# Kaixhin/imitation-learning

Measured on NVIDIA H100. Metric: env_steps_per_s, higher is better.
Workload: dtype f32

## Files before the change

### imitation-learning_b200/csrc/api.cu

```cuda
#include "common.cuh"
#include <cstdlib>

thread_local char g_il_error[512] = "";
int gail_init();
int gmmil_pwil_init();
int gemm_init();
int mlp_init();

extern "C" const char* il_last_error(void) { return g_il_error; }
extern "C" int il_version(void) { return 100; }

extern "C" int il_create(int device, il_handle** out) {
  IL_CHECK(out != nullptr, "il_create: null out");
  int count = 0;
  cudaError_t e = cudaGetDeviceCount(&count);
  if (e != cudaSuccess || count == 0) IL_FAIL("il_create: no CUDA device (%s); this library has no CPU fallback", cudaGetErrorString(e));
  IL_CHECK(device >= 0 && device < count, "il_create: device %d out of range (%d devices)", device, count);
  cudaDeviceProp prop;
  IL_CUDA(cudaGetDeviceProperties(&prop, device));
  IL_CHECK(prop.major == 9 && prop.minor == 0, "il_create: device %d is sm_%d%d; this library is built for sm_90a (H100) only", device, prop.major, prop.minor);
  IL_CUDA(cudaSetDevice(device));
  IL_TRY(gail_init());
  IL_TRY(gmmil_pwil_init());
  IL_TRY(tc_gemm_init());
  IL_TRY(gemm_init());
  IL_TRY(mlp_init());
  il_handle* h = new il_handle();
  h->device = device;
  h->sm_count = prop.multiProcessorCount;
  h->gemm_mode = IL_GEMM_FP32;
  {
    const char* wt = getenv("IL_WIDE_TN");
    h->wide_tn = (wt && wt[0] == '0') ? 0 : 1;
    const char* ff = getenv("IL_FIRST_LAYER_FAST");
    h->first_layer_fast = ff ? atoi(ff) : 2;
    const char* mb = getenv("IL_MASK_BITS");
    h->mask_bits = mb ? atoi(mb) : 2;
    const char* hf = getenv("IL_HEAD_FUSED");
    h->head_fused = (hf && hf[0] == '0') ? 0 : 1;
    const char* ds = getenv("IL_DEBUG_SYNC");
    h->debug_sync = (ds && ds[0] == '1') ? 1 : 0;
    const char* at = getenv("IL_ADAM_TMA");
    h->adam_tma = at ? atoi(at) : 1;
    const char* gt = getenv("IL_GAIL_TILED");
    h->gail_tiled = (gt && gt[0] == '0') ? 0 : 1;
    const char* fl = getenv("IL_TC_FUSE_L1");
    h->tc_fuse_l1 = (fl && fl[0] == '1') ? 1 : 0;
    const char* th = getenv("IL_THIN_HOIST");
    h->thin_hoist = (th && th[0] == '0') ? 0 : 1;
  }
  h->launches = 0;
  h->profiling = 0;
  h->profiled_bytes = 0.0;
  h->eval_graph = nullptr;
  h->build_stream = nullptr;
  *out = h;
  return 0;
}

extern "C" int il_destroy(il_handle* h) {
  if (h) il_eval_release(h);
  if (h && h->build_stream) cudaStreamDestroy(h->build_stream);
  delete h;
  return 0;
}

extern "C" int il_set_gemm_mode(il_handle* h, int mode) {
  IL_CHECK(h, "il_set_gemm_mode: null handle");
  IL_CHECK(mode >= IL_GEMM_FP32 && mode <= IL_GEMM_TF32, "il_set_gemm_mode: bad mode %d", mode);
  h->gemm_mode = mode;
  return 0;
}

extern "C" int64_t il_launch_count(il_handle* h) { return h ? h->launches : -1; }

extern "C" int il_set_option(il_handle* h, const char* name, int value) {
  IL_CHECK(h && name, "il_set_option: null argument");
  if (!strcmp(name, "tc_fuse_l1")) h->tc_fuse_l1 = value;
  else if (!strcmp(name, "gail_tiled")) h->gail_tiled = value;
  else if (!strcmp(name, "adam_tma")) h->adam_tma = value;
  else if (!strcmp(name, "head_fused")) h->head_fused = value;
  else if (!strcmp(name, "mask_bits")) h->mask_bits = value;
  else if (!strcmp(name, "first_layer_fast")) h->first_layer_fast = value;
  else if (!strcmp(name, "wide_tn")) h->wide_tn = value;
  else if (!strcmp(name, "thin_hoist")) h->thin_hoist = value;
  else IL_FAIL("il_set_option: unknown option '%s'", name);
  return 0;
}

extern "C" int il_struct_sizes(int32_t* out) {
  out[0] = (int32_t)sizeof(il_mlp);
  out[1] = (int32_t)sizeof(il_adam);
  out[2] = (int32_t)sizeof(il_batch);
  out[3] = (int32_t)sizeof(il_replay);
  out[4] = (int32_t)sizeof(il_sac_args);
  out[5] = (int32_t)sizeof(il_gail);
  out[6] = (int32_t)sizeof(il_gail_update_args);
  out[7] = (int32_t)sizeof(il_pwil);
  out[8] = (int32_t)sizeof(il_env);
  out[9] = (int32_t)sizeof(il_bc_args);
  out[10] = (int32_t)sizeof(il_eval_args);
  out[11] = (int32_t)sizeof(il_gailx);
  out[12] = (int32_t)sizeof(il_gailx_update_args);
  out[13] = (int32_t)sizeof(il_red);
  out[14] = (int32_t)sizeof(il_red_update_args);
  return 0;
}

extern "C" int il_mlp_param_offsets(const int32_t* dims, int n_layers, int64_t* w_off, int64_t* b_off, int64_t* total) {
  IL_CHECK(dims && n_layers >= 1 && n_layers <= IL_MAX_LAYERS, "il_mlp_param_offsets: bad arguments");
  const MlpOffsets o = mlp_offsets(dims, n_layers);
  for (int l = 0; l < n_layers; ++l) {
    if (w_off) w_off[l] = o.w[l];
    if (b_off) b_off[l] = o.b[l];
  }
  if (total) *total = o.total;
  return 0;
}

extern "C" int il_row_layout(int S, int A, int32_t* off, int32_t* row_len) {
  IL_CHECK(S > 0 && A > 0, "il_row_layout: S=%d A=%d", S, A);
  const RowLayout L = row_layout(S, A);
  if (off) {
    off[0] = L.state; off[1] = L.action; off[2] = L.reward; off[3] = L.next_state;
    off[4] = L.terminal; off[5] = L.timeout; off[6] = L.weight; off[7] = L.step;
  }
  if (row_len) *row_len = L.len;
  return 0;
}

namespace {

__global__ void fill_kernel(float* __restrict__ out, int64_t n, uint64_t seed, uint64_t stream_id, const uint64_t* __restrict__ counter, int normal,
                            const uint64_t* __restrict__ seed_r) {
  const uint64_t base = counter ? *counter : 0ull;
  if (seed_r) { seed = seed_r[blockIdx.y]; out += (int64_t)blockIdx.y * n; }
  const uint2 key = make_uint2((uint32_t)seed, (uint32_t)(seed >> 32));
  for (int64_t q = (int64_t)blockIdx.x * blockDim.x + threadIdx.x; q * 4 < n; q += (int64_t)gridDim.x * blockDim.x) {
    const uint64_t c = base + (uint64_t)q;
    const uint4 r = philox4x32_10(make_uint4((uint32_t)c, (uint32_t)(c >> 32), (uint32_t)stream_id, (uint32_t)(stream_id >> 32)), key);
    float v[4];
    if (normal) {
      const float u0 = 1.f - u32_to_unit(r.x), u1 = u32_to_unit(r.y), u2 = 1.f - u32_to_unit(r.z), u3 = u32_to_unit(r.w);
      const float r0 = sqrtf(-2.f * logf(u0)), r1 = sqrtf(-2.f * logf(u2));
      float s0, c0, s1, c1;
      sincospif(2.f * u1, &s0, &c0);
      sincospif(2.f * u3, &s1, &c1);
      v[0] = r0 * c0; v[1] = r0 * s0; v[2] = r1 * c1; v[3] = r1 * s1;
    } else {
      v[0] = u32_to_unit(r.x); v[1] = u32_to_unit(r.y); v[2] = u32_to_unit(r.z); v[3] = u32_to_unit(r.w);
    }
    for (int j = 0; j < 4; ++j)
      if (q * 4 + j < n) out[q * 4 + j] = v[j];
  }
}

constexpr int BETA_ATTEMPTS = 16;

__device__ float log_gamma_mt(float a, uint64_t c, uint64_t stream_id, uint32_t tag, uint2 key, float* boost_u) {
  const float d = a - 1.f / 3.f, cc = 1.f / sqrtf(9.f * d);
  for (int k = 0; k < BETA_ATTEMPTS; ++k) {
    const uint4 q = philox4x32_10(make_uint4((uint32_t)c, (uint32_t)(c >> 32), (uint32_t)stream_id, (uint32_t)(stream_id >> 32) ^ (tag | (uint32_t)k)), key);
    if (k == 0) *boost_u = 1.f - u32_to_unit(q.w);
    const float x = sqrtf(-2.f * logf(1.f - u32_to_unit(q.x))) * cospif(2.f * u32_to_unit(q.y));
    const float t = fmaf(cc, x, 1.f);
    if (t <= 0.f) continue;
    const float lt = logf(t), v = t * t * t;
    if (logf(1.f - u32_to_unit(q.z)) < 0.5f * x * x + d - d * v + 3.f * d * lt) return logf(d) + 3.f * lt;
  }
  return logf(d);
}

__global__ void beta_fill_kernel(float* __restrict__ out, int64_t total, int64_t n, const float* __restrict__ alpha_r, uint64_t seed, uint64_t stream_id,
                                 const uint64_t* __restrict__ counter, const uint64_t* __restrict__ seed_r) {
  const uint64_t base = counter ? *counter : 0ull;
  if (seed_r) { seed = seed_r[blockIdx.y]; out += (int64_t)blockIdx.y * n; total = n; }
  const uint2 key = make_uint2((uint32_t)seed, (uint32_t)(seed >> 32));
  for (int64_t i = (int64_t)blockIdx.x * blockDim.x + threadIdx.x; i < total; i += (int64_t)gridDim.x * blockDim.x) {
    const uint64_t c = base + (uint64_t)(i >> 2);
    const uint32_t lane = (uint32_t)(i & 3);
    const float alpha = alpha_r[seed_r ? (int64_t)blockIdx.y : i / n];
    float v;
    if (alpha == 1.f) {
      const uint4 q = philox4x32_10(make_uint4((uint32_t)c, (uint32_t)(c >> 32), (uint32_t)stream_id, (uint32_t)(stream_id >> 32)), key);
      v = u32_to_unit(lane == 0 ? q.x : lane == 1 ? q.y : lane == 2 ? q.z : q.w);
    } else if (!(alpha > 0.f)) {
      v = __int_as_float(0x7fc00000);
    } else {
      const float a = alpha < 1.f ? alpha + 1.f : alpha;
      float ux, uy;
      float lx = log_gamma_mt(a, c, stream_id, 0x80000000u | (lane << 5), key, &ux);
      float ly = log_gamma_mt(a, c, stream_id, 0x80000000u | (lane << 5) | 16u, key, &uy);
      if (alpha < 1.f) { lx += logf(ux) / alpha; ly += logf(uy) / alpha; }
      const float t = ly - lx;
      v = t >= 0.f ? 1.f / (1.f + expf(t)) : 1.f - 1.f / (1.f + expf(-t));
    }
    out[i] = v;
  }
}

__global__ void counter_add_kernel(uint64_t* c, uint64_t inc) { *c += inc; }

dim3 rng_grid(il_handle* h, int64_t units, int R) {
  int64_t blocks = (units + 255) / 256;
  const int64_t cap = (int64_t)h->sm_count * 16 / R;
  if (blocks > cap) blocks = cap;
  if (blocks < 1) blocks = 1;
  return dim3((unsigned)blocks, (unsigned)R);
}

int fill(il_handle* h, float* out, int64_t n, uint64_t seed, uint64_t stream_id, const uint64_t* counter, void* stream, int normal) {
  IL_CHECK(h && out && n >= 0, "il_fill: bad argument");
  if (n == 0) return 0;
  int64_t blocks = (n / 4 + 255) / 256;
  if (blocks > (int64_t)h->sm_count * 16) blocks = (int64_t)h->sm_count * 16;
  if (blocks < 1) blocks = 1;
  IL_LAUNCH(h, fill_kernel, (unsigned)blocks, 256, 0, (cudaStream_t)stream, out, n, seed, stream_id, counter, normal, nullptr);
  return 0;
}

int fill_r(il_handle* h, float* out, int R, int64_t n_per_replica, const uint64_t* seed_r, uint64_t stream_id, const uint64_t* counter, void* stream, int normal) {
  IL_CHECK(h && out && seed_r && R > 0 && R <= IL_MAX_GRID_Y && n_per_replica >= 0, "il_fill_%s_r: bad argument (R = %d)", normal ? "normal" : "uniform", R);
  if (n_per_replica == 0) return 0;
  IL_LAUNCH(h, fill_kernel, rng_grid(h, (n_per_replica + 3) / 4, R), 256, 0, (cudaStream_t)stream, out, n_per_replica, 0ull, stream_id, counter, normal, seed_r);
  return 0;
}

}

extern "C" int il_fill_normal(il_handle* h, float* out, int64_t n, uint64_t seed, uint64_t stream_id, const uint64_t* counter, void* stream) {
  return fill(h, out, n, seed, stream_id, counter, stream, 1);
}
extern "C" int il_fill_uniform(il_handle* h, float* out, int64_t n, uint64_t seed, uint64_t stream_id, const uint64_t* counter, void* stream) {
  return fill(h, out, n, seed, stream_id, counter, stream, 0);
}
extern "C" int il_fill_normal_r(il_handle* h, float* out, int R, int64_t n_per_replica, const uint64_t* seed_r, uint64_t stream_id, const uint64_t* counter, void* stream) {
  return fill_r(h, out, R, n_per_replica, seed_r, stream_id, counter, stream, 1);
}
extern "C" int il_fill_uniform_r(il_handle* h, float* out, int R, int64_t n_per_replica, const uint64_t* seed_r, uint64_t stream_id, const uint64_t* counter, void* stream) {
  return fill_r(h, out, R, n_per_replica, seed_r, stream_id, counter, stream, 0);
}
extern "C" int il_fill_beta(il_handle* h, float* out, int R, int64_t n_per_replica, const float* alpha_r, uint64_t seed, uint64_t stream_id, const uint64_t* counter,
                            void* stream) {
  IL_CHECK(h && out && alpha_r && R > 0 && n_per_replica >= 0, "il_fill_beta: bad argument");
  const int64_t total = (int64_t)R * n_per_replica;
  if (total == 0) return 0;
  int64_t blocks = (total + 255) / 256;
  if (blocks > (int64_t)h->sm_count * 16) blocks = (int64_t)h->sm_count * 16;
  IL_LAUNCH(h, beta_fill_kernel, (unsigned)blocks, 256, 0, (cudaStream_t)stream, out, total, n_per_replica, alpha_r, seed, stream_id, counter, nullptr);
  return 0;
}
extern "C" int il_fill_beta_r(il_handle* h, float* out, int R, int64_t n_per_replica, const float* alpha_r, const uint64_t* seed_r, uint64_t stream_id,
                              const uint64_t* counter, void* stream) {
  IL_CHECK(h && out && alpha_r && seed_r && R > 0 && R <= IL_MAX_GRID_Y && n_per_replica >= 0, "il_fill_beta_r: bad argument (R = %d)", R);
  if (n_per_replica == 0) return 0;
  IL_LAUNCH(h, beta_fill_kernel, rng_grid(h, n_per_replica, R), 256, 0, (cudaStream_t)stream, out, n_per_replica, n_per_replica, alpha_r, 0ull, stream_id, counter, seed_r);
  return 0;
}
extern "C" int il_counter_add(il_handle* h, uint64_t* counter, uint64_t inc, void* stream) {
  IL_CHECK(h && counter, "il_counter_add: null argument");
  IL_LAUNCH(h, counter_add_kernel, 1, 1, 0, (cudaStream_t)stream, counter, inc);
  return 0;
}
```

### imitation-learning_b200/csrc/common.cuh

```cuda
#pragma once
#include <cuda_runtime.h>
#include <stdint.h>
#include <stdio.h>
#include <string.h>

#include <vector>

#include "../../include/il_b200.h"

#define IL_MAX_GRID_Y 65535

struct ProfiledLaunch {
  cudaEvent_t start, stop;
  double flops;
  double bytes;
};
struct il_handle {
  int device;
  int sm_count;
  int gemm_mode;
  int thin_hoist;
  int wide_tn;
  int first_layer_fast;
  int mask_bits;
  int head_fused;
  int debug_sync;
  int adam_tma;
  int gail_tiled;
  int tc_fuse_l1;
  long long launches;
  int profiling;
  std::vector<ProfiledLaunch> profiled;
  double profiled_bytes;
  void* eval_graph;
  cudaStream_t build_stream;
};
void il_eval_release(il_handle* h);

extern thread_local char g_il_error[512];

#define IL_FAIL(...)                                     \
  do {                                                   \
    snprintf(g_il_error, sizeof(g_il_error), __VA_ARGS__); \
    return 1;                                            \
  } while (0)

#define IL_CHECK(cond, ...)        \
  do {                             \
    if (!(cond)) IL_FAIL(__VA_ARGS__); \
  } while (0)

#define IL_CUDA(expr)                                                                             \
  do {                                                                                            \
    cudaError_t _e = (expr);                                                                      \
    if (_e != cudaSuccess) IL_FAIL("%s failed: %s (%s:%d)", #expr, cudaGetErrorString(_e), __FILE__, __LINE__); \
  } while (0)

#define IL_LAUNCH(h, kernel, grid, block, smem, stream, ...)                                      \
  do {                                                                                            \
    kernel<<<(grid), (block), (smem), (cudaStream_t)(stream)>>>(__VA_ARGS__);                     \
    (h)->launches++;                                                                              \
    cudaError_t _e = cudaPeekAtLastError();                                                       \
    if (_e != cudaSuccess) IL_FAIL("launch of %s failed: %s (%s:%d)", #kernel, cudaGetErrorString(_e), __FILE__, __LINE__); \
  } while (0)

#define IL_TRY(expr)          \
  do {                        \
    int _r = (expr);          \
    if (_r != 0) return _r;   \
  } while (0)

__host__ __device__ static inline int64_t il_align_up(int64_t x, int64_t a) { return (x + a - 1) / a * a; }

struct RowLayout {
  int state, action, reward, next_state, terminal, timeout, weight, step, len;
};
__host__ __device__ inline RowLayout row_layout(int S, int A) {
  RowLayout L;
  L.state = 0;
  L.action = S;
  L.reward = S + A;
  L.next_state = S + A + 1;
  L.terminal = 2 * S + A + 1;
  L.timeout = L.terminal + 1;
  L.weight = L.terminal + 2;
  L.step = L.terminal + 3;
  L.len = (2 * S + A + 5 + 3) / 4 * 4;
  return L;
}

struct MlpOffsets {
  int64_t w[IL_MAX_LAYERS], b[IL_MAX_LAYERS], total;
};
__host__ __device__ static inline MlpOffsets mlp_offsets(const int32_t* dims, int n_layers) {
  MlpOffsets o;
  int64_t off = 0;
  for (int l = 0; l < n_layers; ++l) {
    o.w[l] = off;
    off = il_align_up(off + (int64_t)dims[l + 1] * dims[l], 4);
    o.b[l] = off;
    off = il_align_up(off + dims[l + 1], 4);
  }
  o.total = il_align_up(off, 32);
  return o;
}

__device__ __forceinline__ float act_apply(float x, int act) {
  if (act == IL_ACT_RELU) return fmaxf(x, 0.f);
  if (act == IL_ACT_TANH) return tanhf(x);
  return 1.f / (1.f + expf(-x));
}
__device__ __forceinline__ float act_grad_from_output(float y, int act) {
  if (act == IL_ACT_RELU) return y > 0.f ? 1.f : 0.f;
  if (act == IL_ACT_TANH) return 1.f - y * y;
  return y * (1.f - y);
}
__device__ __forceinline__ float softplusf(float x) {
  return x > 20.f ? x : log1pf(expf(x));
}
__device__ __forceinline__ float sigmoidf(float x) { return 1.f / (1.f + expf(-x)); }

__device__ __forceinline__ float warp_sum(float v) {
#pragma unroll
  for (int o = 16; o > 0; o >>= 1) v += __shfl_xor_sync(0xffffffffu, v, o);
  return v;
}
__device__ __forceinline__ float warp_max(float v) {
#pragma unroll
  for (int o = 16; o > 0; o >>= 1) v = fmaxf(v, __shfl_xor_sync(0xffffffffu, v, o));
  return v;
}
__device__ __forceinline__ float block_sum(float v, float* red) {
  const int lane = threadIdx.x & 31, warp = threadIdx.x >> 5, nw = (blockDim.x + 31) >> 5;
  v = warp_sum(v);
  __syncthreads();
  if (lane == 0) red[warp] = v;
  __syncthreads();
  float r = 0.f;
  if (warp == 0) {
    r = lane < nw ? red[lane] : 0.f;
    r = warp_sum(r);
    if (lane == 0) red[0] = r;
  }
  __syncthreads();
  return red[0];
}

__device__ __forceinline__ uint4 philox4x32_10(uint4 ctr, uint2 key) {
  const uint32_t M0 = 0xD2511F53u, M1 = 0xCD9E8D57u, W0 = 0x9E3779B9u, W1 = 0xBB67AE85u;
#pragma unroll
  for (int i = 0; i < 10; ++i) {
    const uint32_t hi0 = __umulhi(M0, ctr.x), lo0 = M0 * ctr.x;
    const uint32_t hi1 = __umulhi(M1, ctr.z), lo1 = M1 * ctr.z;
    ctr = make_uint4(hi1 ^ ctr.y ^ key.x, lo1, hi0 ^ ctr.w ^ key.y, lo0);
    key.x += W0;
    key.y += W1;
  }
  return ctr;
}
__device__ __forceinline__ float u32_to_unit(uint32_t x) { return (float)(x >> 8) * (1.0f / 16777216.0f); }

struct GemmArgs {
  const float* A;
  int64_t a_gs;
  int a_gdiv, lda, a_kmajor;
  const float* B;
  int64_t b_gs;
  int b_gdiv, ldb, b_kmajor;
  float* C;
  int64_t c_gs;
  int ldc;
  const float* bias;
  int64_t bias_gs;
  int act;
  const float* mask;
  int64_t mask_gs;
  int ldmask, mask_act;
  float* colsum;
  int64_t colsum_gs;
  int accumulate;
  int M, N, K, G;
  const uint32_t* mask_bits;
  int64_t mask_bits_gs;
  uint32_t* bits_out;
  int64_t bits_out_gs;
};
int launch_gemm(il_handle* h, const GemmArgs& a, cudaStream_t stream);
bool gemm_uses_tc(const il_handle* h, const GemmArgs& a);
bool gemm_first_layer_emits_bits(const il_handle* h, const GemmArgs& a);
double gemm_algorithmic_bytes(const GemmArgs& a, bool stores_c);
int profile_open(il_handle* h, ProfiledLaunch* pl, double flops, double bytes, cudaStream_t stream);
int profile_close(il_handle* h, ProfiledLaunch* pl, cudaStream_t stream);

bool tc_gemm_eligible(const GemmArgs& a);
int launch_tc_gemm(il_handle* h, const GemmArgs& a, cudaStream_t stream);
int tc_gemm_init();
struct TcFuseL1 {
  const float* x;
  int64_t x_gs;
  int x_gdiv, x_ld, x_k;
  const float* w1;
  const float* b1;
  int64_t gs;
  float* store;
  int64_t store_gs;
};
bool tc_head_fusable(const il_handle* h, const GemmArgs& a, int head_n);
bool tc_l1_fusable(const il_handle* h, const GemmArgs& a, int x_k);
bool tc_dx_head_fusable(const il_handle* h, const GemmArgs& a, int head_n);
int launch_tc_gemm_dx_head(il_handle* h, const GemmArgs& a, const float* w, int64_t w_gs, int w_ns, int head_n, float* out, int64_t out_gs, cudaStream_t stream);
int launch_tc_gemm_head(il_handle* h, const GemmArgs& a, const float* head_w, const float* head_b, int64_t head_gs, int head_n, float* head_out, int64_t head_out_gs, int store_c,
                        cudaStream_t stream, const TcFuseL1* l1 = nullptr);
```

### imitation-learning_b200/csrc/mlp.cu

```cuda
#include "mlp.cuh"

#include <math.h>

constexpr int HB_MAXN = 8;
struct HeadBwdArgs {
  const float* dout; int64_t dout_gs; int dout_gdiv, ld_dout;
  const float* w; int64_t w_gs;
  const float* y; int64_t y_gs;
  float* dz; int64_t dz_gs;
  float* dw; float* db; float* db_prev; int64_t g_gs;
  int n, H, Nh;
};
int launch_head_backward(il_handle* h, const HeadBwdArgs& a, int G, cudaStream_t stream);
int launch_head_dx_bits(il_handle* h, const HeadBwdArgs& a, const uint32_t* bits, int64_t bits_gs, int G, cudaStream_t stream);

int mlp_validate(const il_mlp* m, const char* what) {
  IL_CHECK(m != nullptr && m->params != nullptr, "%s: null mlp", what);
  IL_CHECK(m->n_layers >= 1 && m->n_layers <= IL_MAX_LAYERS, "%s: n_layers %d out of range", what, m->n_layers);
  IL_CHECK(m->activation >= 0 && m->activation <= 2, "%s: bad activation %d", what, m->activation);
  for (int l = 0; l <= m->n_layers; ++l) IL_CHECK(m->dims[l] > 0, "%s: dims[%d] = %d", what, l, m->dims[l]);
  const MlpOffsets o = mlp_offsets(m->dims, m->n_layers);
  IL_CHECK(m->stride >= o.total - 31 && m->stride % 4 == 0, "%s: stride %lld too small / unaligned for %lld parameters", what, (long long)m->stride, (long long)o.total);
  IL_CHECK((reinterpret_cast<uintptr_t>(m->params) & 15) == 0, "%s: params not 16-byte aligned", what);
  return 0;
}

int mlp_max_hidden(const il_mlp* m) {
  int mx = 1;
  for (int l = 1; l <= m->n_layers; ++l) mx = m->dims[l] > mx ? m->dims[l] : mx;
  return mx;
}

static int64_t mlp_bits_bytes(const il_mlp* m, int G, int n, int l) {
  return m->dims[l + 1] % 32 == 0 ? il_align_up((int64_t)G * n * (m->dims[l + 1] / 32) * 4, 256) : 0;
}

int64_t mlp_acts_bytes(const il_mlp* m, int G, int n) {
  int64_t b = 0;
  for (int l = 0; l + 1 < m->n_layers; ++l) b += il_align_up((int64_t)G * n * m->dims[l + 1] * 4, 256) + mlp_bits_bytes(m, G, n, l);
  return b;
}

char* mlp_acts_carve(const il_mlp* m, int G, int n, char* ws, MlpActs* acts) {
  for (int l = 0; l < IL_MAX_LAYERS; ++l) { acts->hid[l] = nullptr; acts->bits[l] = nullptr; acts->bits_valid[l] = false; }
  for (int l = 0; l + 1 < m->n_layers; ++l) {
    acts->hid[l] = reinterpret_cast<float*>(ws);
    ws += il_align_up((int64_t)G * n * m->dims[l + 1] * 4, 256);
    if (mlp_bits_bytes(m, G, n, l)) {
      acts->bits[l] = reinterpret_cast<uint32_t*>(ws);
      ws += mlp_bits_bytes(m, G, n, l);
    }
  }
  return ws;
}

int mlp_forward(il_handle* h, const il_mlp* m, int G, int n, MatView X, MlpActs& acts, float* out, int64_t out_gs, int ld_out, cudaStream_t stream, int keep) {
  const MlpOffsets o = mlp_offsets(m->dims, m->n_layers);
  const int L = m->n_layers;
  const bool keep_hidden = keep != MLP_KEEP_NONE;
  const bool want_bits = h->mask_bits && keep_hidden && m->activation == IL_ACT_RELU;
  for (int l = 0; l < IL_MAX_LAYERS; ++l) acts.bits_valid[l] = false;
  auto layer_args = [&](int l) {
    GemmArgs a{};
    if (l == 0) { a.A = X.ptr; a.a_gs = X.gs; a.a_gdiv = X.gdiv; a.lda = X.ld; }
    else { a.A = acts.hid[l - 1]; a.a_gs = (int64_t)n * m->dims[l]; a.a_gdiv = 1; a.lda = m->dims[l]; }
    a.a_kmajor = 1;
    a.B = m->params + o.w[l]; a.b_gs = m->stride; a.b_gdiv = 1; a.ldb = m->dims[l]; a.b_kmajor = 1;
    a.bias = m->params + o.b[l]; a.bias_gs = m->stride;
    if (l == L - 1) { a.C = out; a.c_gs = out_gs; a.ldc = ld_out; a.act = -1; }
    else { a.C = acts.hid[l]; a.c_gs = (int64_t)n * m->dims[l + 1]; a.ldc = m->dims[l + 1]; a.act = m->activation; }
    a.M = n; a.N = m->dims[l + 1]; a.K = m->dims[l]; a.G = G;
    return a;
  };
  const bool head_shape = L >= 2 && m->activation == IL_ACT_RELU && ld_out == m->dims[L] && out_gs == (int64_t)n * m->dims[L];
  for (int l = 0; l < L; ++l) {
    if (head_shape && l == L - 2) {
      GemmArgs a = layer_args(l);
      if (tc_head_fusable(h, a, m->dims[L])) {
        const bool bits = want_bits && keep == MLP_KEEP_MASKS && acts.bits[l] && m->dims[L] <= HB_MAXN;
        if (bits) { a.bits_out = acts.bits[l]; a.bits_out_gs = (int64_t)n * (m->dims[l + 1] / 32); acts.bits_valid[l] = true; }
        IL_TRY(launch_tc_gemm_head(h, a, m->params + o.w[L - 1], m->params + o.b[L - 1], m->stride, m->dims[L], out, out_gs, keep_hidden && !bits ? 1 : 0, stream));
        return 0;
      }
    }
    if (head_shape && l == 0 && L == 3) {
      GemmArgs a1 = layer_args(1);
      a1.A = nullptr; a1.a_gs = 0; a1.a_gdiv = 1; a1.lda = m->dims[1];
      if (tc_head_fusable(h, a1, m->dims[L]) && tc_l1_fusable(h, a1, m->dims[0])) {
        TcFuseL1 f{};
        f.x = X.ptr; f.x_gs = X.gs; f.x_gdiv = X.gdiv; f.x_ld = X.ld; f.x_k = m->dims[0];
        f.w1 = m->params + o.w[0]; f.b1 = m->params + o.b[0]; f.gs = m->stride;
        f.store = keep_hidden ? acts.hid[0] : nullptr; f.store_gs = (int64_t)n * m->dims[1];
        IL_TRY(launch_tc_gemm_head(h, a1, m->params + o.w[L - 1], m->params + o.b[L - 1], m->stride, m->dims[L], out, out_gs, keep_hidden ? 1 : 0, stream, &f));
        return 0;
      }
    }
    GemmArgs a = layer_args(l);
    if (want_bits && l + 1 < L && acts.bits[l] && gemm_first_layer_emits_bits(h, a)) {
      a.bits_out = acts.bits[l]; a.bits_out_gs = (int64_t)n * (m->dims[l + 1] / 32);
      acts.bits_valid[l] = true;
    }
    IL_TRY(launch_gemm(h, a, stream));
  }
  return 0;
}

static bool head_backward_eligible(const il_mlp* m, int n, int64_t grad_stride) {
  const int L = m->n_layers, H = m->dims[L - 1], Nh = m->dims[L];
  return m->activation == IL_ACT_RELU && Nh <= HB_MAXN && H % 4 == 0 && n <= 1024 && grad_stride % 4 == 0 && m->stride % 4 == 0;
}

int mlp_backward(il_handle* h, const il_mlp* m, int G, int n, MatView X, const MlpActs& acts, MatView dOut, float* grads, int64_t grad_stride,
                 float* dX, int64_t dx_gs, int ld_dx, int dx_col0, int dx_cols, float* tmpA, float* tmpB, cudaStream_t stream) {
  const MlpOffsets o = mlp_offsets(m->dims, m->n_layers);
  const int L = m->n_layers;
  MatView dZ = dOut;
  float* next_tmp = tmpA;
  bool bias_done = false;
  for (int l = L - 1; l >= 0; --l) {
    MatView Xin = l == 0 ? X : MatView{acts.hid[l - 1], (int64_t)n * m->dims[l], 1, m->dims[l]};
    if (l == L - 1 && l > 0 && grads && h->head_fused && head_backward_eligible(m, n, grad_stride)) {
      HeadBwdArgs a{};
      a.dout = dZ.ptr; a.dout_gs = dZ.gs; a.dout_gdiv = dZ.gdiv; a.ld_dout = dZ.ld;
      a.w = m->params + o.w[l]; a.w_gs = m->stride;
      a.y = acts.hid[l - 1]; a.y_gs = (int64_t)n * m->dims[l];
      a.dz = next_tmp; a.dz_gs = (int64_t)n * m->dims[l];
      a.dw = grads + o.w[l]; a.db = grads + o.b[l]; a.db_prev = grads + o.b[l - 1]; a.g_gs = grad_stride;
      a.n = n; a.H = m->dims[l]; a.Nh = m->dims[l + 1];
      IL_TRY(launch_head_backward(h, a, G, stream));
      dZ = MatView{next_tmp, (int64_t)n * m->dims[l], 1, m->dims[l]};
      next_tmp = next_tmp == tmpA ? tmpB : tmpA;
      bias_done = true;
      continue;
    }
    if (l == L - 1 && l > 0 && !grads && acts.bits_valid[l - 1] && m->dims[l + 1] <= HB_MAXN) {
      HeadBwdArgs a{};
      a.dout = dZ.ptr; a.dout_gs = dZ.gs; a.dout_gdiv = dZ.gdiv; a.ld_dout = dZ.ld;
      a.w = m->params + o.w[l]; a.w_gs = m->stride;
      a.dz = next_tmp; a.dz_gs = (int64_t)n * m->dims[l];
      a.n = n; a.H = m->dims[l]; a.Nh = m->dims[l + 1];
      IL_TRY(launch_head_dx_bits(h, a, acts.bits[l - 1], (int64_t)n * (m->dims[l] / 32), G, stream));
      dZ = MatView{next_tmp, (int64_t)n * m->dims[l], 1, m->dims[l]};
      next_tmp = next_tmp == tmpA ? tmpB : tmpA;
      continue;
    }
    if (grads) {
      GemmArgs a{};
      a.A = dZ.ptr; a.a_gs = dZ.gs; a.a_gdiv = dZ.gdiv; a.lda = dZ.ld; a.a_kmajor = 0;
      a.B = Xin.ptr; a.b_gs = Xin.gs; a.b_gdiv = Xin.gdiv; a.ldb = Xin.ld; a.b_kmajor = 0;
      a.C = grads + o.w[l]; a.c_gs = grad_stride; a.ldc = m->dims[l]; a.act = -1;
      if (!bias_done) { a.colsum = grads + o.b[l]; a.colsum_gs = grad_stride; }
      bias_done = false;
      a.M = m->dims[l + 1]; a.N = m->dims[l]; a.K = n; a.G = G;
      IL_TRY(launch_gemm(h, a, stream));
    }
    if (l > 0) {
      GemmArgs a{};
      a.A = dZ.ptr; a.a_gs = dZ.gs; a.a_gdiv = dZ.gdiv; a.lda = dZ.ld; a.a_kmajor = 1;
      a.B = m->params + o.w[l]; a.b_gs = m->stride; a.b_gdiv = 1; a.ldb = m->dims[l]; a.b_kmajor = 0;
      a.C = next_tmp; a.c_gs = (int64_t)n * m->dims[l]; a.ldc = m->dims[l]; a.act = -1;
      a.mask_act = m->activation;
      a.M = n; a.N = m->dims[l]; a.K = m->dims[l + 1]; a.G = G;
      if (acts.bits_valid[l - 1] && m->activation == IL_ACT_RELU && gemm_uses_tc(h, a)) {
        a.mask_bits = acts.bits[l - 1]; a.mask_bits_gs = (int64_t)n * (m->dims[l] / 32);
        if (h->mask_bits >= 2 && l == 1 && !grads && dX && ld_dx == dx_cols && dx_gs == (int64_t)n * dx_cols && tc_dx_head_fusable(h, a, dx_cols)) {
          a.C = nullptr;
          IL_TRY(launch_tc_gemm_dx_head(h, a, m->params + o.w[0] + dx_col0, m->stride, m->dims[0], dx_cols, dX, dx_gs, stream));
          return 0;
        }
      } else {
        a.mask = acts.hid[l - 1]; a.mask_gs = (int64_t)n * m->dims[l]; a.ldmask = m->dims[l];
      }
      IL_TRY(launch_gemm(h, a, stream));
      dZ = MatView{next_tmp, (int64_t)n * m->dims[l], 1, m->dims[l]};
      next_tmp = next_tmp == tmpA ? tmpB : tmpA;
    } else if (dX) {
      GemmArgs a{};
      a.A = dZ.ptr; a.a_gs = dZ.gs; a.a_gdiv = dZ.gdiv; a.lda = dZ.ld; a.a_kmajor = 1;
      a.B = m->params + o.w[0] + dx_col0; a.b_gs = m->stride; a.b_gdiv = 1; a.ldb = m->dims[0]; a.b_kmajor = 0;
      a.C = dX; a.c_gs = dx_gs; a.ldc = ld_dx; a.act = -1;
      a.M = n; a.N = dx_cols; a.K = m->dims[1]; a.G = G;
      IL_TRY(launch_gemm(h, a, stream));
    }
  }
  return 0;
}

namespace {

__global__ void actor_head_kernel(const HeadFwdArgs p) {
  const int64_t row = (int64_t)blockIdx.x * blockDim.x + threadIdx.x;
  if (row >= (int64_t)p.R * p.n) return;
  const int r = (int)(row / p.n), i = (int)(row % p.n);
  const int A = p.A;
  const float* hd = p.head + row * 2 * A;
  float* act_row = p.action ? p.action + (int64_t)r * p.action_rs + (int64_t)i * p.ld_action : nullptr;
  if (p.copy_src && act_row) {
    const float* src = p.copy_src + (int64_t)r * p.copy_rs + (int64_t)i * p.copy_ld;
    for (int j = 0; j < p.copy_cols; ++j) act_row[j - p.copy_cols] = __ldg(src + j);
  }
  const float keep = p.zero_mask ? 1.f - __ldg(p.zero_mask + (int64_t)r * p.zero_mask_rs + (int64_t)i * p.zero_mask_ld) : 1.f;
  const float LOG_SQRT_2PI = 0.91893853320467274178f, LOG2 = 0.69314718055994530942f;
  const float A_LO = (float)(-1.0 + 1e-6), A_HI = (float)(1.0 - 1e-6);
  float sum_ladj = 0.f, sum_nlp = 0.f;
  const bool want_lp = p.log_prob != nullptr && (p.eps != nullptr || p.given != nullptr);
  for (int j = 0; j < A; ++j) {
    const float mu = hd[j];
    const float ls = fminf(fmaxf(hd[A + j], -20.f), 2.f);
    if (p.mean) p.mean[row * A + j] = mu;
    if (p.log_std) p.log_std[row * A + j] = ls;
    float x, a;
    const float sd = expf(ls);
    if (p.given) {
      a = fminf(fmaxf(p.given[row * A + j], A_LO), A_HI);
      x = atanhf(a);
    } else if (p.eps) {
      x = __fadd_rn(mu, __fmul_rn(sd, p.eps[row * A + j]));
      a = tanhf(x);
    } else {
      x = mu;
      a = tanhf(mu);
    }
    if (act_row && !p.given) act_row[j] = keep * a;
    if (want_lp) {
      const float var = __fmul_rn(sd, sd);
      const float diff = __fsub_rn(x, mu);
      float nlp = __fdiv_rn(-__fmul_rn(diff, diff), __fmul_rn(2.f, var));
      nlp = __fsub_rn(__fsub_rn(nlp, logf(sd)), LOG_SQRT_2PI);
      const float ladj = __fmul_rn(2.f, __fsub_rn(__fsub_rn(LOG2, x), softplusf(__fmul_rn(-2.f, x))));
      sum_nlp += nlp;
      sum_ladj += ladj;
    }
  }
  if (want_lp) p.log_prob[row] = __fadd_rn(__fsub_rn(0.f, sum_ladj), sum_nlp);
}

struct SmallFwdArgs {
  il_mlp m;
  MlpOffsets o;
  const float* X;
  int64_t x_gs;
  int x_gdiv, ldx, n, maxd;
  float* out;
  int tanh_first;
};
template <int NR>
__global__ void __launch_bounds__(256) mlp_small_forward_kernel(const SmallFwdArgs p) {
  extern __shared__ __align__(16) float sm[];
  const int g = blockIdx.x, r0 = blockIdx.y * NR, tid = threadIdx.x, warp = tid >> 5, lane = tid & 31;
  const int nr = min(NR, p.n - r0), L = p.m.n_layers, maxd = p.maxd;
  float* bufs[2] = {sm, sm + NR * maxd};
  const float* X = p.X + (int64_t)(g / p.x_gdiv) * p.x_gs;
  for (int idx = tid; idx < NR * p.m.dims[0]; idx += 256) {
    const int r = idx / p.m.dims[0], k = idx % p.m.dims[0];
    bufs[0][r * maxd + k] = r < nr ? __ldg(X + (int64_t)(r0 + r) * p.ldx + k) : 0.f;
  }
  const float* prm = p.m.params + (int64_t)g * p.m.stride;
  __syncthreads();
  for (int l = 0; l < L; ++l) {
    const int in = p.m.dims[l], od = p.m.dims[l + 1];
    const float* W = prm + p.o.w[l];
    const float* bias = prm + p.o.b[l];
    const float* xin = bufs[l & 1];
    float* xout = bufs[(l + 1) & 1];
    const bool vec = (in % 4 == 0) && (p.m.stride % 4 == 0);
    if (NR == 1 && vec && in <= 16) {
      for (int o = tid; o < od; o += 256) {
        const float4* wr = reinterpret_cast<const float4*>(W + (int64_t)o * in);
        float4 w4[4];
#pragma unroll
        for (int q = 0; q < 4; ++q) w4[q] = 4 * q < in ? __ldg(wr + q) : make_float4(0.f, 0.f, 0.f, 0.f);
        float v = __ldg(bias + o);
#pragma unroll
        for (int q = 0; q < 4; ++q)
          if (4 * q < in) {
            const float4 x4 = *reinterpret_cast<const float4*>(xin + 4 * q);
            v = fmaf(w4[q].x, x4.x, fmaf(w4[q].y, x4.y, fmaf(w4[q].z, x4.z, fmaf(w4[q].w, x4.w, v))));
          }
        if (l < L - 1) v = act_apply(v, p.m.activation);
        xout[o] = v;
      }
      __syncthreads();
      continue;
    }
    if (NR == 1 && vec && in % 128 == 0 && in <= 256) {
      const int kv = in >> 7;
      float4 x4[2];
#pragma unroll
      for (int v = 0; v < 2; ++v) x4[v] = v < kv ? *reinterpret_cast<const float4*>(xin + v * 128 + lane * 4) : make_float4(0.f, 0.f, 0.f, 0.f);
      for (int o0 = warp * 8; o0 < od; o0 += 64) {
        float4 w4[8][2];
#pragma unroll
        for (int u = 0; u < 8; ++u)
#pragma unroll
          for (int v = 0; v < 2; ++v)
            w4[u][v] = (o0 + u < od && v < kv) ? __ldg(reinterpret_cast<const float4*>(W + (int64_t)(o0 + u) * in + v * 128 + lane * 4)) : make_float4(0.f, 0.f, 0.f, 0.f);
        float a8[8];
#pragma unroll
        for (int u = 0; u < 8; ++u) {
          float t = 0.f;
#pragma unroll
          for (int v = 0; v < 2; ++v) t = fmaf(w4[u][v].x, x4[v].x, fmaf(w4[u][v].y, x4[v].y, fmaf(w4[u][v].z, x4[v].z, fmaf(w4[u][v].w, x4[v].w, t))));
          a8[u] = warp_sum(t);
        }
        if (lane < 8 && o0 + lane < od) {
          float v = a8[0];
#pragma unroll
          for (int u = 1; u < 8; ++u) v = lane == u ? a8[u] : v;
          v += __ldg(bias + o0 + lane);
          if (l < L - 1) v = act_apply(v, p.m.activation);
          xout[o0 + lane] = v;
        }
      }
      __syncthreads();
      continue;
    }
    if (NR == 1 && vec) {
      for (int o0 = warp * 4; o0 < od; o0 += 32) {
        float a4[4] = {0.f, 0.f, 0.f, 0.f};
        for (int k = lane * 4; k < in; k += 128) {
          const float4 x4 = *reinterpret_cast<const float4*>(xin + k);
          float4 w4[4];
#pragma unroll
          for (int u = 0; u < 4; ++u) w4[u] = o0 + u < od ? __ldg(reinterpret_cast<const float4*>(W + (int64_t)(o0 + u) * in + k)) : make_float4(0.f, 0.f, 0.f, 0.f);
#pragma unroll
          for (int u = 0; u < 4; ++u) a4[u] = fmaf(w4[u].x, x4.x, fmaf(w4[u].y, x4.y, fmaf(w4[u].z, x4.z, fmaf(w4[u].w, x4.w, a4[u]))));
        }
#pragma unroll
        for (int u = 0; u < 4; ++u) a4[u] = warp_sum(a4[u]);
        if (lane < 4 && o0 + lane < od) {
          float v = (lane == 0 ? a4[0] : lane == 1 ? a4[1] : lane == 2 ? a4[2] : a4[3]) + __ldg(bias + o0 + lane);
          if (l < L - 1) v = act_apply(v, p.m.activation);
          xout[o0 + lane] = v;
        }
      }
      __syncthreads();
      continue;
    }
    for (int o = warp; o < od; o += 8) {
      float acc[NR];
#pragma unroll
      for (int r = 0; r < NR; ++r) acc[r] = 0.f;
      const float* wr = W + (int64_t)o * in;
      if (vec) {
        for (int k = lane * 4; k < in; k += 128) {
          const float4 w4 = __ldg(reinterpret_cast<const float4*>(wr + k));
#pragma unroll
          for (int r = 0; r < NR; ++r) {
            const float4 x4 = *reinterpret_cast<const float4*>(xin + r * maxd + k);
            acc[r] = fmaf(w4.x, x4.x, fmaf(w4.y, x4.y, fmaf(w4.z, x4.z, fmaf(w4.w, x4.w, acc[r]))));
          }
        }
      } else {
        for (int k = lane; k < in; k += 32) {
          const float w = __ldg(wr + k);
#pragma unroll
          for (int r = 0; r < NR; ++r) acc[r] = fmaf(w, xin[r * maxd + k], acc[r]);
        }
      }
#pragma unroll
      for (int r = 0; r < NR; ++r) acc[r] = warp_sum(acc[r]);
      if (lane == 0) {
        const float b = __ldg(bias + o);
#pragma unroll
        for (int r = 0; r < NR; ++r) {
          float v = acc[r] + b;
          if (l < L - 1) v = act_apply(v, p.m.activation);
          xout[r * maxd + o] = v;
        }
      }
    }
    __syncthreads();
  }
  const int od = p.m.dims[L];
  const float* fin = bufs[L & 1];
  if (p.tanh_first > 0) {
    const int A = p.tanh_first;
    for (int idx = tid; idx < nr * A; idx += 256) {
      const int r = idx / A, o = idx % A;
      p.out[((int64_t)g * p.n + r0 + r) * A + o] = tanhf(fin[r * maxd + o]);
    }
    return;
  }
  for (int idx = tid; idx < nr * od; idx += 256) {
    const int r = idx / od, o = idx % od;
    p.out[((int64_t)g * p.n + r0 + r) * od + o] = fin[r * maxd + o];
  }
}

struct AdamReplicas {
  const double* lr_r;
  const double* wd_r;
  const float* tau_r;
  int64_t rf;
  float inv_rf;
  int R;
};
struct AdamCoef { float step_size, decay, tau, one_minus_tau; };
constexpr int ADAM_MAX_REPLICAS = 2048;
__device__ __forceinline__ void adam_fill_table(AdamCoef* tab, const AdamReplicas& rp, double lr, double wd, double beta1_d, const int64_t* step, float tau) {
  if (!rp.R) return;
  const double bc1 = 1.0 - pow(beta1_d, (double)*step);
  for (int r = threadIdx.x; r < rp.R; r += blockDim.x) {
    const double l = rp.lr_r ? rp.lr_r[r] : lr, w = rp.wd_r ? rp.wd_r[r] : wd;
    const float t = rp.tau_r ? rp.tau_r[r] : tau;
    tab[r] = AdamCoef{(float)(l / bc1), w != 0.0 ? (float)(1.0 - l * w) : 1.f, t, (float)(1.0 - (double)t)};
  }
}
__device__ __forceinline__ int adam_replica(int64_t f, const AdamReplicas& rp) {
  int r = (int)((float)f * rp.inv_rf);
  if ((int64_t)r * rp.rf > f) --r;
  else if ((int64_t)(r + 1) * rp.rf <= f) ++r;
  return r;
}

__global__ void adam_kernel(float* __restrict__ p, const float* __restrict__ g, float* __restrict__ m, float* __restrict__ v, const int64_t* __restrict__ step,
                            double lr, double beta1_d, double beta2_d, double eps_d, double wd, int64_t n, float* __restrict__ target, float tau, float one_minus_tau,
                            const AdamReplicas rp) {
  extern __shared__ AdamCoef adam_tab[];
  __shared__ float s_step_size, s_bc2_sqrt;
  if (threadIdx.x == 0) {
    const double t = (double)*step;
    const double bc1 = 1.0 - pow(beta1_d, t), bc2 = 1.0 - pow(beta2_d, t);
    s_step_size = (float)(lr / bc1);
    s_bc2_sqrt = (float)sqrt(bc2);
  }
  adam_fill_table(adam_tab, rp, lr, wd, beta1_d, step, tau);
  __syncthreads();
  const float step_size = s_step_size, bc2_sqrt = s_bc2_sqrt;
  const float decay = (float)(1.0 - lr * wd), w1 = (float)(1.0 - beta1_d), w2 = (float)(1.0 - beta2_d);
  const float beta2 = (float)beta2_d, eps = (float)eps_d;
  const bool has_wd = wd != 0.0;
  auto upd = [&](float& pi, float& mi, float& vi, float gi, float ss, float dc, bool wdf) {
    if (wdf) pi = __fmul_rn(pi, dc);
    mi = __fadd_rn(mi, __fmul_rn(w1, __fsub_rn(gi, mi)));
    vi = __fadd_rn(__fmul_rn(vi, beta2), __fmul_rn(__fmul_rn(w2, gi), gi));
    const float denom = __fadd_rn(__fdiv_rn(sqrtf(vi), bc2_sqrt), eps);
    pi = __fadd_rn(pi, __fmul_rn(-ss, __fdiv_rn(mi, denom)));
  };
  const int64_t n4 = n >> 2;
  for (int64_t i = (int64_t)blockIdx.x * blockDim.x + threadIdx.x; i < n4; i += (int64_t)gridDim.x * blockDim.x) {
    float ss = step_size, dc = decay, ta = tau, omt = one_minus_tau;
    bool wdf = has_wd;
    if (rp.R) {
      const AdamCoef c = adam_tab[adam_replica(i << 2, rp)];
      ss = c.step_size; dc = c.decay; wdf = c.decay != 1.f; ta = c.tau; omt = c.one_minus_tau;
    }
    float4 pv = reinterpret_cast<float4*>(p)[i], mv = reinterpret_cast<float4*>(m)[i], vv = reinterpret_cast<float4*>(v)[i];
    const float4 gv = reinterpret_cast<const float4*>(g)[i];
    upd(pv.x, mv.x, vv.x, gv.x, ss, dc, wdf); upd(pv.y, mv.y, vv.y, gv.y, ss, dc, wdf); upd(pv.z, mv.z, vv.z, gv.z, ss, dc, wdf); upd(pv.w, mv.w, vv.w, gv.w, ss, dc, wdf);
    reinterpret_cast<float4*>(p)[i] = pv; reinterpret_cast<float4*>(m)[i] = mv; reinterpret_cast<float4*>(v)[i] = vv;
    if (target) {
      const float tau = ta, one_minus_tau = omt;
      float4 tv = reinterpret_cast<float4*>(target)[i];
      tv.x = __fadd_rn(__fmul_rn(tv.x, tau), __fmul_rn(one_minus_tau, pv.x)); tv.y = __fadd_rn(__fmul_rn(tv.y, tau), __fmul_rn(one_minus_tau, pv.y));
      tv.z = __fadd_rn(__fmul_rn(tv.z, tau), __fmul_rn(one_minus_tau, pv.z)); tv.w = __fadd_rn(__fmul_rn(tv.w, tau), __fmul_rn(one_minus_tau, pv.w));
      reinterpret_cast<float4*>(target)[i] = tv;
    }
  }
  for (int64_t i = (n4 << 2) + (int64_t)blockIdx.x * blockDim.x + threadIdx.x; i < n; i += (int64_t)gridDim.x * blockDim.x) {
    float pi = p[i], mi = m[i], vi = v[i];
    upd(pi, mi, vi, g[i], step_size, decay, has_wd);
    p[i] = pi; m[i] = mi; v[i] = vi;
    if (target) target[i] = __fadd_rn(__fmul_rn(target[i], tau), __fmul_rn(one_minus_tau, pi));
  }
}

constexpr int ADAM_STREAMS = 5;
constexpr int ADAM_CONSUMERS = 256;
template <int TILE, int STAGES> constexpr int adam_tma_smem() { return STAGES * ADAM_STREAMS * TILE * 4 + 2 * STAGES * 8 + 64; }
__device__ __forceinline__ void adam_mbar_wait(uint32_t bar, uint32_t parity) {
  asm volatile(
      "{\n\t.reg .pred q;\n\t"
      "ADAM_WAIT:\n\t"
      "mbarrier.try_wait.parity.shared::cta.b64 q, [%0], %1;\n\t"
      "@q bra ADAM_DONE;\n\t"
      "bra ADAM_WAIT;\n\t"
      "ADAM_DONE:\n\t}" ::"r"(bar), "r"(parity) : "memory");
}
template <int TILE, int STAGES>
__global__ void __launch_bounds__(ADAM_CONSUMERS + 32) adam_tma_kernel(float* __restrict__ p, const float* __restrict__ g, float* __restrict__ m, float* __restrict__ v,
                                                                      const int64_t* __restrict__ step, double lr, double beta1_d, double beta2_d, double eps_d, double wd, int64_t n,
                                                                      float* __restrict__ target, float tau, float one_minus_tau, const AdamReplicas rp) {
  extern __shared__ __align__(128) uint8_t adam_smem[];
  float* buf = reinterpret_cast<float*>(adam_smem);
  AdamCoef* tab = reinterpret_cast<AdamCoef*>(adam_smem + adam_tma_smem<TILE, STAGES>());
  const uint32_t smem0 = (uint32_t)__cvta_generic_to_shared(buf);
  const uint32_t full0 = smem0 + (uint32_t)(STAGES * ADAM_STREAMS * TILE * 4), done0 = full0 + 8u * STAGES;
  __shared__ float s_step_size, s_bc2_sqrt;
  const int tid = threadIdx.x;
  adam_fill_table(tab, rp, lr, wd, beta1_d, step, tau);
  if (tid == 0) {
    const double t = (double)*step;
    s_step_size = (float)(lr / (1.0 - pow(beta1_d, t)));
    s_bc2_sqrt = (float)sqrt(1.0 - pow(beta2_d, t));
    for (int s_ = 0; s_ < STAGES; ++s_) {
      asm volatile("mbarrier.init.shared::cta.b64 [%0], 1;" ::"r"(full0 + 8u * s_));
      asm volatile("mbarrier.init.shared::cta.b64 [%0], %1;" ::"r"(done0 + 8u * s_), "r"(ADAM_CONSUMERS));
    }
    asm volatile("fence.mbarrier_init.release.cluster;" ::: "memory");
  }
  __syncthreads();
  const int64_t n_tiles = (n + TILE - 1) / TILE;
  const int n_streams = target ? 5 : 4;
  auto tile_floats = [&](int64_t tile) { const int64_t left = n - tile * TILE; return (int)(left < TILE ? left : TILE); };
  const int64_t my_tiles = blockIdx.x < n_tiles ? (n_tiles - blockIdx.x + gridDim.x - 1) / gridDim.x : 0;
  if (tid >= ADAM_CONSUMERS) {
    if (tid != ADAM_CONSUMERS) return;
    auto issue_loads = [&](int64_t k) {
      const int64_t tile = blockIdx.x + k * gridDim.x;
      const int stage = (int)(k % STAGES);
      const uint32_t bytes = (uint32_t)tile_floats(tile) * 4u, bar = full0 + 8u * stage;
      asm volatile("mbarrier.arrive.expect_tx.shared::cta.b64 _, [%0], %1;" ::"r"(bar), "r"(bytes * (uint32_t)n_streams) : "memory");
      const float* src[5] = {p, g, m, v, target};
      for (int q = 0; q < n_streams; ++q)
        asm volatile("cp.async.bulk.shared::cluster.global.mbarrier::complete_tx::bytes [%0], [%1], %2, [%3];" ::"r"(smem0 + (uint32_t)((stage * ADAM_STREAMS + q) * TILE * 4)),
                     "l"(src[q] + tile * TILE), "r"(bytes), "r"(bar) : "memory");
    };
    for (int64_t k = 0; k < STAGES - 1 && k < my_tiles; ++k) issue_loads(k);
    for (int64_t k = 0; k < my_tiles; ++k) {
      const int stage = (int)(k % STAGES);
      const int64_t tile = blockIdx.x + k * gridDim.x;
      if (k + STAGES - 1 < my_tiles) {
        if (k > 0) asm volatile("cp.async.bulk.wait_group.read 0;" ::: "memory");
        issue_loads(k + STAGES - 1);
      }
      adam_mbar_wait(done0 + 8u * stage, (uint32_t)((k / STAGES) & 1));
      const uint32_t bytes = (uint32_t)tile_floats(tile) * 4u;
      float* dst[5] = {p, nullptr, m, v, target};
      for (int q = 0; q < n_streams; ++q) {
        if (!dst[q]) continue;
        asm volatile("cp.async.bulk.global.shared::cta.bulk_group [%0], [%1], %2;" ::"l"(dst[q] + tile * TILE), "r"(smem0 + (uint32_t)((stage * ADAM_STREAMS + q) * TILE * 4)), "r"(bytes)
                     : "memory");
      }
      asm volatile("cp.async.bulk.commit_group;" ::: "memory");
    }
    asm volatile("cp.async.bulk.wait_group 0;" ::: "memory");
    return;
  }
  const float step_size = s_step_size, bc2_sqrt = s_bc2_sqrt;
  const float decay = (float)(1.0 - lr * wd), w1 = (float)(1.0 - beta1_d), w2 = (float)(1.0 - beta2_d), beta2 = (float)beta2_d, eps = (float)eps_d;
  const bool has_wd = wd != 0.0;
  auto upd = [&](float& pi, float& mi, float& vi, float gi, float ss, float dc, bool wdf) {
    if (wdf) pi = __fmul_rn(pi, dc);
    mi = __fadd_rn(mi, __fmul_rn(w1, __fsub_rn(gi, mi)));
    vi = __fadd_rn(__fmul_rn(vi, beta2), __fmul_rn(__fmul_rn(w2, gi), gi));
    const float denom = __fadd_rn(__fdiv_rn(sqrtf(vi), bc2_sqrt), eps);
    pi = __fadd_rn(pi, __fmul_rn(-ss, __fdiv_rn(mi, denom)));
  };
  for (int64_t k = 0; k < my_tiles; ++k) {
    const int stage = (int)(k % STAGES);
    const int64_t tile = blockIdx.x + k * gridDim.x;
    adam_mbar_wait(full0 + 8u * stage, (uint32_t)((k / STAGES) & 1));
    const int nf4 = tile_floats(tile) >> 2;
    float4* sp = reinterpret_cast<float4*>(buf + (stage * ADAM_STREAMS + 0) * TILE);
    const float4* sg = reinterpret_cast<const float4*>(buf + (stage * ADAM_STREAMS + 1) * TILE);
    float4* smm = reinterpret_cast<float4*>(buf + (stage * ADAM_STREAMS + 2) * TILE);
    float4* sv = reinterpret_cast<float4*>(buf + (stage * ADAM_STREAMS + 3) * TILE);
    float4* stg = reinterpret_cast<float4*>(buf + (stage * ADAM_STREAMS + 4) * TILE);
    for (int i = tid; i < nf4; i += ADAM_CONSUMERS) {
      float ss = step_size, dc = decay, ta = tau, omt = one_minus_tau;
      bool wdf = has_wd;
      if (rp.R) {
        const AdamCoef c = tab[adam_replica(tile * TILE + 4 * i, rp)];
        ss = c.step_size; dc = c.decay; wdf = c.decay != 1.f; ta = c.tau; omt = c.one_minus_tau;
      }
      float4 pv = sp[i], mv = smm[i], vv = sv[i];
      const float4 gv = sg[i];
      upd(pv.x, mv.x, vv.x, gv.x, ss, dc, wdf); upd(pv.y, mv.y, vv.y, gv.y, ss, dc, wdf); upd(pv.z, mv.z, vv.z, gv.z, ss, dc, wdf); upd(pv.w, mv.w, vv.w, gv.w, ss, dc, wdf);
      sp[i] = pv; smm[i] = mv; sv[i] = vv;
      if (target) {
        const float tau = ta, one_minus_tau = omt;
        float4 tv = stg[i];
        tv.x = __fadd_rn(__fmul_rn(tv.x, tau), __fmul_rn(one_minus_tau, pv.x)); tv.y = __fadd_rn(__fmul_rn(tv.y, tau), __fmul_rn(one_minus_tau, pv.y));
        tv.z = __fadd_rn(__fmul_rn(tv.z, tau), __fmul_rn(one_minus_tau, pv.z)); tv.w = __fadd_rn(__fmul_rn(tv.w, tau), __fmul_rn(one_minus_tau, pv.w));
        stg[i] = tv;
      }
    }
    asm volatile("fence.proxy.async.shared::cta;" ::: "memory");
    asm volatile("mbarrier.arrive.shared::cta.b64 _, [%0];" ::"r"(done0 + 8u * stage) : "memory");
  }
}

template <int TILE, int STAGES>
static int launch_adam_tma(il_handle* h, int ctas_per_sm, float* params, const float* grads, const il_adam* opt, int64_t n, cudaStream_t stream, float* polyak_target, float polyak_factor,
                           const AdamReplicas& rp) {
  static bool attr_set = false;
  if (!attr_set) {
    IL_CUDA(cudaFuncSetAttribute(adam_tma_kernel<TILE, STAGES>, cudaFuncAttributeMaxDynamicSharedMemorySize, adam_tma_smem<TILE, STAGES>() + ADAM_MAX_REPLICAS * (int)sizeof(AdamCoef)));
    attr_set = true;
  }
  const size_t smem = (size_t)adam_tma_smem<TILE, STAGES>() + (size_t)rp.R * sizeof(AdamCoef);
  IL_LAUNCH(h, (adam_tma_kernel<TILE, STAGES>), h->sm_count * ctas_per_sm, ADAM_CONSUMERS + 32, smem, stream, params, grads, opt->m, opt->v, opt->step, opt->lr, opt->beta1,
            opt->beta2, opt->eps, opt->weight_decay, n, polyak_target, polyak_factor, (float)(1.0 - (double)polyak_factor), rp);
  return 0;
}
constexpr int ADAM_TMA_MIN_TILES = 4096;


template <int NH>
__global__ void __launch_bounds__(256, 2) head_backward_kernel(const HeadBwdArgs p) {
  extern __shared__ __align__(16) float hb_sm[];
  const int g = blockIdx.y, n0 = blockIdx.x * 256, tid = threadIdx.x, tc = tid & 63, tr = tid >> 6, col = n0 + tc * 4;
  float* dos = hb_sm;
  float* red = hb_sm + p.n * HB_MAXN;
  const float* dout = p.dout + (int64_t)(g / p.dout_gdiv) * p.dout_gs;
  const bool active = col < p.H;
  const float* Y = p.y + (int64_t)g * p.y_gs + col;
  float4 yv[4], yn[4];
  auto fetch = [&](float4 (&dst)[4], int b0) {
#pragma unroll
    for (int u = 0; u < 4; ++u) {
      const int b = b0 + 4 * u;
      dst[u] = (active && b < p.n) ? __ldg(reinterpret_cast<const float4*>(Y + (int64_t)b * p.H)) : make_float4(0.f, 0.f, 0.f, 0.f);
    }
  };
  fetch(yv, tr);
  for (int i = tid; i < p.n * HB_MAXN; i += 256) {
    const int b = i / HB_MAXN, j = i % HB_MAXN;
    dos[i] = j < p.Nh ? __ldg(dout + (int64_t)b * p.ld_dout + j) : 0.f;
  }
  float4 w[NH];
#pragma unroll
  for (int j = 0; j < NH; ++j) w[j] = (active && j < p.Nh) ? __ldg(reinterpret_cast<const float4*>(p.w + (int64_t)g * p.w_gs + (int64_t)j * p.H + col)) : make_float4(0.f, 0.f, 0.f, 0.f);
  __syncthreads();
  float4 dw[NH], cs = make_float4(0.f, 0.f, 0.f, 0.f);
#pragma unroll
  for (int j = 0; j < NH; ++j) dw[j] = make_float4(0.f, 0.f, 0.f, 0.f);
  if (active) {
    float* DZ = p.dz + (int64_t)g * p.dz_gs + col;
    for (int b0 = tr; b0 < p.n; b0 += 16) {
      fetch(yn, b0 + 16);
#pragma unroll
      for (int u = 0; u < 4; ++u) {
        const int b = b0 + 4 * u;
        if (b >= p.n) continue;
        float dj[NH];
        if (NH == 1) dj[0] = dos[b * HB_MAXN];
        else {
          const float4 d0 = *reinterpret_cast<const float4*>(dos + b * HB_MAXN), d1 = *reinterpret_cast<const float4*>(dos + b * HB_MAXN + 4);
          const float t[8] = {d0.x, d0.y, d0.z, d0.w, d1.x, d1.y, d1.z, d1.w};
#pragma unroll
          for (int j = 0; j < NH; ++j) dj[j] = t[j];
        }
        float4 z = make_float4(0.f, 0.f, 0.f, 0.f);
#pragma unroll
        for (int j = 0; j < NH; ++j) {
          z.x = fmaf(dj[j], w[j].x, z.x); z.y = fmaf(dj[j], w[j].y, z.y); z.z = fmaf(dj[j], w[j].z, z.z); z.w = fmaf(dj[j], w[j].w, z.w);
          dw[j].x = fmaf(dj[j], yv[u].x, dw[j].x); dw[j].y = fmaf(dj[j], yv[u].y, dw[j].y); dw[j].z = fmaf(dj[j], yv[u].z, dw[j].z); dw[j].w = fmaf(dj[j], yv[u].w, dw[j].w);
        }
        z.x = yv[u].x > 0.f ? z.x : 0.f; z.y = yv[u].y > 0.f ? z.y : 0.f; z.z = yv[u].z > 0.f ? z.z : 0.f; z.w = yv[u].w > 0.f ? z.w : 0.f;
        cs.x += z.x; cs.y += z.y; cs.z += z.z; cs.w += z.w;
        *reinterpret_cast<float4*>(DZ + (int64_t)b * p.H) = z;
      }
#pragma unroll
      for (int u = 0; u < 4; ++u) yv[u] = yn[u];
    }
  }
  float4* r4 = reinterpret_cast<float4*>(red);
#pragma unroll
  for (int j = 0; j < NH; ++j) r4[(tr * (HB_MAXN + 1) + j) * 64 + tc] = dw[j];
  r4[(tr * (HB_MAXN + 1) + HB_MAXN) * 64 + tc] = cs;
  __syncthreads();
  if (tr == 0 && active) {
#pragma unroll
    for (int j = 0; j <= HB_MAXN; ++j) {
      if ((j < NH && j < p.Nh) || j == HB_MAXN) {
        float4 a = r4[(0 * (HB_MAXN + 1) + j) * 64 + tc];
#pragma unroll
        for (int q = 1; q < 4; ++q) {
          const float4 t = r4[(q * (HB_MAXN + 1) + j) * 64 + tc];
          a.x += t.x; a.y += t.y; a.z += t.z; a.w += t.w;
        }
        float* dst = j == HB_MAXN ? p.db_prev + (int64_t)g * p.g_gs + col : p.dw + (int64_t)g * p.g_gs + (int64_t)j * p.H + col;
        *reinterpret_cast<float4*>(dst) = a;
      }
    }
  }
  if (blockIdx.x == 0 && tid < p.Nh) {
    float sacc = 0.f;
    for (int b = 0; b < p.n; ++b) sacc += dos[b * HB_MAXN + tid];
    p.db[(int64_t)g * p.g_gs + tid] = sacc;
  }
}

__global__ void tick_kernel(int64_t* s0, int64_t* s1, int64_t* s2) {
  if (s0) *s0 += 1;
  if (s1) *s1 += 1;
  if (s2) *s2 += 1;
}

__global__ void polyak_kernel(float* __restrict__ t, const float* __restrict__ o, int64_t n, float tau, float one_minus_tau) {
  for (int64_t i = (int64_t)blockIdx.x * blockDim.x + threadIdx.x; i < n; i += (int64_t)gridDim.x * blockDim.x)
    t[i] = __fadd_rn(__fmul_rn(t[i], tau), __fmul_rn(one_minus_tau, o[i]));
}

__global__ void split_twin_kernel(const float* __restrict__ q, float* __restrict__ q1, float* __restrict__ q2, int R, int n) {
  const int64_t i = (int64_t)blockIdx.x * blockDim.x + threadIdx.x;
  if (i >= (int64_t)R * n) return;
  const int r = (int)(i / n), b = (int)(i % n);
  if (q1) q1[i] = q[((int64_t)2 * r) * n + b];
  if (q2) q2[i] = q[((int64_t)2 * r + 1) * n + b];
}

__global__ void concat_kernel(const float* __restrict__ s, int64_t s_rs, int ld_s, int S, const float* __restrict__ a, int64_t a_rs, int ld_a, int A,
                              float* __restrict__ x, int R, int n) {
  const int64_t idx = (int64_t)blockIdx.x * blockDim.x + threadIdx.x;
  const int d = S + A;
  if (idx >= (int64_t)R * n * d) return;
  const int j = (int)(idx % d);
  const int64_t row = idx / d;
  const int r = (int)(row / n), i = (int)(row % n);
  x[idx] = j < S ? s[(int64_t)r * s_rs + (int64_t)i * ld_s + j] : a[(int64_t)r * a_rs + (int64_t)i * ld_a + (j - S)];
}

inline int ew_blocks(int64_t n, int threads, int sm_count) {
  int64_t b = (n + threads - 1) / threads;
  const int64_t cap = (int64_t)sm_count * 16;
  return (int)(b < 1 ? 1 : (b > cap ? cap : b));
}

}

int launch_actor_head(il_handle* h, const HeadFwdArgs& a, cudaStream_t stream) {
  const int64_t rows = (int64_t)a.R * a.n;
  IL_LAUNCH(h, actor_head_kernel, (unsigned)((rows + 127) / 128), 128, 0, stream, a);
  return 0;
}

int launch_adam(il_handle* h, float* params, const float* grads, const il_adam* opt, int64_t n, cudaStream_t stream, float* polyak_target, float polyak_factor,
                const float* polyak_r) {
  IL_CHECK(opt->m && opt->v && opt->step, "adam: null state");
  IL_CHECK(((reinterpret_cast<uintptr_t>(params) | reinterpret_cast<uintptr_t>(grads) | reinterpret_cast<uintptr_t>(opt->m) | reinterpret_cast<uintptr_t>(opt->v) |
             reinterpret_cast<uintptr_t>(polyak_target)) & 15) == 0, "adam: buffers must be 16-byte aligned");
  AdamReplicas rp{opt->lr_r, opt->weight_decay_r, polyak_target ? polyak_r : nullptr, 0, 0.f, 0};
  if (rp.lr_r || rp.wd_r || rp.tau_r) {
    const int64_t rf = opt->replica_floats;
    IL_CHECK(rf > 0 && rf % 4 == 0 && n % rf == 0, "adam: per-replica hyper-parameters need replica_floats (%lld) > 0, a multiple of 4 dividing n = %lld", (long long)rf, (long long)n);
    IL_CHECK(n / rf <= ADAM_MAX_REPLICAS, "adam: %lld replicas with per-replica hyper-parameters exceed the limit of %d per buffer", (long long)(n / rf), ADAM_MAX_REPLICAS);
    rp.rf = rf; rp.inv_rf = 1.f / (float)rf; rp.R = (int)(n / rf);
  }
  if (h->adam_tma && n % 4 == 0 && n >= (int64_t)ADAM_TMA_MIN_TILES * h->sm_count * 2) {
    const int variant = h->adam_tma;
    switch (variant) {
      case 2: return launch_adam_tma<4096, 2>(h, 1, params, grads, opt, n, stream, polyak_target, polyak_factor, rp);
      case 3: return launch_adam_tma<2048, 3>(h, 1, params, grads, opt, n, stream, polyak_target, polyak_factor, rp);
      case 4: return launch_adam_tma<1024, 4>(h, 2, params, grads, opt, n, stream, polyak_target, polyak_factor, rp);
      case 5: return launch_adam_tma<1024, 3>(h, 3, params, grads, opt, n, stream, polyak_target, polyak_factor, rp);
      case 6: return launch_adam_tma<512, 4>(h, 4, params, grads, opt, n, stream, polyak_target, polyak_factor, rp);
      case 7: return launch_adam_tma<2048, 4>(h, 1, params, grads, opt, n, stream, polyak_target, polyak_factor, rp);
      default: return launch_adam_tma<2048, 2>(h, 2, params, grads, opt, n, stream, polyak_target, polyak_factor, rp);
    }
  }
  IL_LAUNCH(h, adam_kernel, ew_blocks(n / 4 + 1, 256, h->sm_count), 256, (size_t)rp.R * sizeof(AdamCoef), stream, params, grads, opt->m, opt->v, opt->step, opt->lr, opt->beta1, opt->beta2,
            opt->eps, opt->weight_decay, n, polyak_target, polyak_factor, (float)(1.0 - (double)polyak_factor), rp);
  return 0;
}

namespace {
template <int NH, int U>
__global__ void __launch_bounds__(256) head_dx_bits_kernel(const HeadBwdArgs p, const uint32_t* __restrict__ bits, int64_t bits_gs) {
  const int g = blockIdx.y, tid = threadIdx.x, tc = tid & 63, tr = tid >> 6, col = blockIdx.x * 256 + tc * 4;
  if (col >= p.H) return;
  const float* __restrict__ dout = p.dout + (int64_t)(g / p.dout_gdiv) * p.dout_gs;
  const uint32_t* __restrict__ bw = bits + (int64_t)g * bits_gs + (col >> 5);
  const int sh = col & 31, wpr = p.H >> 5;
  float4 w[NH];
#pragma unroll
  for (int j = 0; j < NH; ++j) w[j] = j < p.Nh ? __ldg(reinterpret_cast<const float4*>(p.w + (int64_t)g * p.w_gs + (int64_t)j * p.H + col)) : make_float4(0.f, 0.f, 0.f, 0.f);
  float* __restrict__ dz = p.dz + (int64_t)g * p.dz_gs + col;
  for (int b0 = tr; b0 < p.n; b0 += 4 * U) {
    uint32_t m[U];
    float d[U][NH];
#pragma unroll
    for (int u = 0; u < U; ++u) {
      const int b = b0 + 4 * u;
      m[u] = b < p.n ? __ldg(bw + (int64_t)b * wpr) >> sh : 0u;
#pragma unroll
      for (int j = 0; j < NH; ++j) d[u][j] = (j < p.Nh && b < p.n) ? __ldg(dout + (int64_t)b * p.ld_dout + j) : 0.f;
    }
#pragma unroll
    for (int u = 0; u < U; ++u) {
      const int b = b0 + 4 * u;
      if (b >= p.n) break;
      float4 v = make_float4(0.f, 0.f, 0.f, 0.f);
#pragma unroll
      for (int j = 0; j < NH; ++j)
        if (j < p.Nh) { v.x = fmaf(d[u][j], w[j].x, v.x); v.y = fmaf(d[u][j], w[j].y, v.y); v.z = fmaf(d[u][j], w[j].z, v.z); v.w = fmaf(d[u][j], w[j].w, v.w); }
      v.x = m[u] & 1u ? v.x : 0.f; v.y = m[u] & 2u ? v.y : 0.f; v.z = m[u] & 4u ? v.z : 0.f; v.w = m[u] & 8u ? v.w : 0.f;
      *reinterpret_cast<float4*>(dz + (int64_t)b * p.H) = v;
    }
  }
}
}

int launch_head_dx_bits(il_handle* h, const HeadBwdArgs& a, const uint32_t* bits, int64_t bits_gs, int G, cudaStream_t stream) {
  IL_CHECK(a.H % 32 == 0 && a.Nh <= HB_MAXN && (reinterpret_cast<uintptr_t>(a.w) & 15) == 0 && a.w_gs % 4 == 0 && (reinterpret_cast<uintptr_t>(a.dz) & 15) == 0 && a.dz_gs % 4 == 0,
           "head_dx_bits: H=%d Nh=%d or unaligned buffers", a.H, a.Nh);
  if (a.Nh == 1) IL_LAUNCH(h, (head_dx_bits_kernel<1, 8>), dim3((a.H + 255) / 256, G), 256, 0, stream, a, bits, bits_gs);
  else IL_LAUNCH(h, (head_dx_bits_kernel<HB_MAXN, 4>), dim3((a.H + 255) / 256, G), 256, 0, stream, a, bits, bits_gs);
  return 0;
}

int launch_head_backward(il_handle* h, const HeadBwdArgs& a, int G, cudaStream_t stream) {
  const size_t smem = ((size_t)a.n * HB_MAXN + 4 * (HB_MAXN + 1) * 64 * 4) * sizeof(float);
  if (a.Nh == 1) IL_LAUNCH(h, head_backward_kernel<1>, dim3((a.H + 255) / 256, G), 256, smem, stream, a);
  else IL_LAUNCH(h, head_backward_kernel<HB_MAXN>, dim3((a.H + 255) / 256, G), 256, smem, stream, a);
  return 0;
}

int mlp_init() {
  IL_CUDA(cudaFuncSetAttribute(head_backward_kernel<1>, cudaFuncAttributeMaxDynamicSharedMemorySize, (1024 * HB_MAXN + 4 * (HB_MAXN + 1) * 64 * 4) * 4));
  IL_CUDA(cudaFuncSetAttribute(head_backward_kernel<HB_MAXN>, cudaFuncAttributeMaxDynamicSharedMemorySize, (1024 * HB_MAXN + 4 * (HB_MAXN + 1) * 64 * 4) * 4));
  return 0;
}

int launch_tick(il_handle* h, int64_t* s0, int64_t* s1, int64_t* s2, cudaStream_t stream) {
  IL_LAUNCH(h, tick_kernel, 1, 1, 0, stream, s0, s1, s2);
  return 0;
}

int mlp_small_forward(il_handle* h, const il_mlp* m, int G, int n, MatView X, float* out, cudaStream_t stream, int tanh_first) {
  SmallFwdArgs a;
  a.m = *m; a.o = mlp_offsets(m->dims, m->n_layers);
  a.X = X.ptr; a.x_gs = X.gs; a.x_gdiv = X.gdiv; a.ldx = X.ld; a.n = n; a.out = out; a.tanh_first = tanh_first;
  int maxd = 4;
  for (int l = 0; l <= m->n_layers; ++l) maxd = m->dims[l] > maxd ? m->dims[l] : maxd;
  a.maxd = (maxd + 3) / 4 * 4;
  if (n == 1) {
    IL_LAUNCH(h, mlp_small_forward_kernel<1>, dim3(G, 1), 256, (size_t)2 * 1 * a.maxd * 4, stream, a);
  } else {
    IL_CHECK((size_t)2 * 8 * a.maxd * 4 <= 48 * 1024, "mlp_small_forward: layer width %d too large", maxd);
    IL_LAUNCH(h, mlp_small_forward_kernel<8>, dim3(G, (n + 7) / 8), 256, (size_t)2 * 8 * a.maxd * 4, stream, a);
  }
  return 0;
}

extern "C" int il_adam_step(il_handle* h, float* params, const float* grads, const il_adam* opt, int64_t n, void* stream) {
  IL_CHECK(h && params && grads && opt, "il_adam_step: null argument");
  IL_TRY(launch_tick(h, opt->step, nullptr, nullptr, (cudaStream_t)stream));
  return launch_adam(h, params, grads, opt, n, (cudaStream_t)stream);
}

extern "C" int il_adam_step_polyak(il_handle* h, float* params, const float* grads, const il_adam* opt, int64_t n, float* target, float polyak_factor, void* stream) {
  IL_CHECK(h && params && grads && opt && target, "il_adam_step_polyak: null argument");
  IL_TRY(launch_tick(h, opt->step, nullptr, nullptr, (cudaStream_t)stream));
  return launch_adam(h, params, grads, opt, n, (cudaStream_t)stream, target, polyak_factor);
}

extern "C" int il_adam_step_polyak_r(il_handle* h, float* params, const float* grads, const il_adam* opt, int64_t n, float* target, const float* polyak_r, void* stream) {
  IL_CHECK(h && params && grads && opt && target && polyak_r, "il_adam_step_polyak_r: null argument");
  IL_TRY(launch_tick(h, opt->step, nullptr, nullptr, (cudaStream_t)stream));
  return launch_adam(h, params, grads, opt, n, (cudaStream_t)stream, target, 0.f, polyak_r);
}

extern "C" int il_polyak(il_handle* h, float* target, const float* online, int64_t n, float polyak_factor, void* stream) {
  IL_CHECK(h && target && online && n >= 0, "il_polyak: bad argument");
  if (n == 0) return 0;
  IL_LAUNCH(h, polyak_kernel, ew_blocks(n, 256, h->sm_count), 256, 0, (cudaStream_t)stream, target, online, n, polyak_factor, (float)(1.0 - (double)polyak_factor));
  return 0;
}

extern "C" int64_t il_actor_workspace_bytes(const il_mlp* actor, int R, int n) {
  return mlp_acts_bytes(actor, R, n) + il_align_up((int64_t)R * n * actor->dims[actor->n_layers] * 4, 256);
}

extern "C" int il_actor_forward(il_handle* h, const il_mlp* actor, int R, int n, const float* states, int64_t states_rs, int ld_states, const float* eps,
                                const float* given_action, float* action, float* log_prob, float* mean, float* log_std, void* workspace, int64_t workspace_bytes,
                                void* stream) {
  IL_CHECK(h && states && workspace, "il_actor_forward: null argument");
  IL_TRY(mlp_validate(actor, "il_actor_forward"));
  IL_CHECK(R > 0 && n > 0, "il_actor_forward: R=%d n=%d", R, n);
  const int out = actor->dims[actor->n_layers];
  IL_CHECK(out % 2 == 0, "il_actor_forward: head size %d is not 2*A", out);
  IL_CHECK(workspace_bytes >= il_actor_workspace_bytes(actor, R, n), "il_actor_forward: workspace too small");
  MlpActs acts;
  char* ws = mlp_acts_carve(actor, R, n, static_cast<char*>(workspace), &acts);
  float* head = reinterpret_cast<float*>(ws);
  if (n <= 32) IL_TRY(mlp_small_forward(h, actor, R, n, MatView{states, states_rs, 1, ld_states}, head, (cudaStream_t)stream));
  else IL_TRY(mlp_forward(h, actor, R, n, MatView{states, states_rs, 1, ld_states}, acts, head, (int64_t)n * out, out, (cudaStream_t)stream, MLP_KEEP_NONE));
  HeadFwdArgs a{};
  a.head = head; a.eps = eps; a.given = given_action;
  a.action = action; a.action_rs = (int64_t)n * (out / 2); a.ld_action = out / 2;
  a.log_prob = log_prob; a.mean = mean; a.log_std = log_std;
  a.R = R; a.n = n; a.A = out / 2;
  return launch_actor_head(h, a, (cudaStream_t)stream);
}

extern "C" int64_t il_critic_workspace_bytes(const il_mlp* critic, int R, int n) {
  return mlp_acts_bytes(critic, 2 * R, n) + il_align_up((int64_t)R * n * critic->dims[0] * 4, 256) + il_align_up((int64_t)2 * R * n * 4, 256);
}

extern "C" int il_critic_forward(il_handle* h, const il_mlp* twin, int R, int n, int S, const float* states, int64_t states_rs, int ld_states, const float* actions,
                                 int64_t actions_rs, int ld_actions, float* q1, float* q2, void* workspace, int64_t workspace_bytes, void* stream) {
  IL_CHECK(h && states && actions && workspace, "il_critic_forward: null argument");
  IL_TRY(mlp_validate(twin, "il_critic_forward"));
  IL_CHECK(twin->dims[twin->n_layers] == 1, "il_critic_forward: critic head must have one output");
  IL_CHECK(workspace_bytes >= il_critic_workspace_bytes(twin, R, n), "il_critic_forward: workspace too small");
  cudaStream_t st = (cudaStream_t)stream;
  const int d = twin->dims[0];
  MlpActs acts;
  char* ws = mlp_acts_carve(twin, 2 * R, n, static_cast<char*>(workspace), &acts);
  float* X = reinterpret_cast<float*>(ws);
  ws += il_align_up((int64_t)R * n * d * 4, 256);
  float* q = reinterpret_cast<float*>(ws);
  const int A = d - S;
  IL_CHECK(S > 0 && A > 0, "il_critic_forward: S=%d with input width %d", S, d);
  const int64_t total = (int64_t)R * n * d;
  IL_LAUNCH(h, concat_kernel, (unsigned)((total + 255) / 256), 256, 0, st, states, states_rs, ld_states, S, actions, actions_rs, ld_actions, A, X, R, n);
  IL_TRY(mlp_forward(h, twin, 2 * R, n, MatView{X, (int64_t)n * d, 2, d}, acts, q, (int64_t)n, 1, st, MLP_KEEP_NONE));
  IL_LAUNCH(h, split_twin_kernel, (unsigned)(((int64_t)R * n + 255) / 256), 256, 0, st, q, q1, q2, R, n);
  return 0;
}
```

### imitation-learning_b200/csrc/tc_gemm.cu

```cuda
#include "common.cuh"
#include <cstdio>
#include <cstdlib>

namespace {

constexpr int BM = 128, BN = 256, BK = 16;
constexpr int PRODUCER_THREADS = 128, CONSUMER_THREADS = 256;
constexpr int THREADS = PRODUCER_THREADS + CONSUMER_THREADS;
constexpr int LAUNCH_REGS = 168;
constexpr int producer_regs(bool fuse) { return fuse ? 72 : 56; }
constexpr int consumer_regs(bool fuse) { return (THREADS * LAUNCH_REGS - PRODUCER_THREADS * producer_regs(fuse)) / CONSUMER_THREADS; }
static_assert(THREADS * LAUNCH_REGS <= 65536 && consumer_regs(false) % 8 == 0 && consumer_regs(true) % 8 == 0, "tc_gemm: setmaxnreg split");
constexpr int CONSUMER_BAR = 1, PRODUCER_BAR = 2;
constexpr int A_BYTES = BM * BK * 4, B_BYTES = BN * BK * 4;
constexpr int A_HI = 0, A_LO = A_BYTES, B_HI = 2 * A_BYTES, B_LO = 2 * A_BYTES + B_BYTES;
constexpr int STAGE_BYTES = 2 * (A_BYTES + B_BYTES);
constexpr int N_STAGES = 3;
constexpr int RAW_STAGES = 3;
constexpr int HEAD_MAX = 8;
constexpr int HEAD_BYTES = (BN + HEAD_MAX * BN) * 4;
constexpr int L1_MAXK = 16, L1_ROWS = 256;
constexpr int L1_W_BYTES = L1_ROWS * L1_MAXK * 4, L1_B_BYTES = L1_ROWS * 4, L1_X_BYTES = BM * L1_MAXK * 4;
constexpr int raw_a_bytes(bool fuse) { return fuse ? 0 : A_BYTES; }
constexpr int raw_bytes(bool fuse) { return raw_a_bytes(fuse) + B_BYTES; }
constexpr int RAW_OFF = N_STAGES * STAGE_BYTES;
constexpr int head_off(bool fuse) { return RAW_OFF + RAW_STAGES * raw_bytes(fuse); }
constexpr int l1_off(bool fuse) { return head_off(fuse) + HEAD_BYTES; }
constexpr int BAR_BYTES = 64;
static_assert(2 * N_STAGES * 8 <= BAR_BYTES && BAR_BYTES + 512 - 16 <= 1024, "tc_gemm: mbarrier area");
constexpr int smem_bytes(bool fuse) { return 1024 + l1_off(fuse) + (fuse ? L1_W_BYTES + L1_B_BYTES + L1_X_BYTES : 0); }
static_assert(smem_bytes(false) <= 227 * 1024 && smem_bytes(true) <= 227 * 1024, "tc_gemm: shared memory over the 227 KB per-CTA limit");

__device__ __forceinline__ uint32_t smem_u32(const void* p) { return (uint32_t)__cvta_generic_to_shared(p); }
__device__ __forceinline__ void fence_proxy_async() { asm volatile("fence.proxy.async.shared::cta;" ::: "memory"); }
__device__ __forceinline__ void wgmma_fence() { asm volatile("wgmma.fence.sync.aligned;" ::: "memory"); }
__device__ __forceinline__ void wgmma_commit() { asm volatile("wgmma.commit_group.sync.aligned;" ::: "memory"); }
template <int N>
__device__ __forceinline__ void wgmma_wait() { asm volatile("wgmma.wait_group.sync.aligned %0;" ::"n"(N) : "memory"); }
__device__ __forceinline__ void cp_async16(uint32_t dst, const float* src) { asm volatile("cp.async.cg.shared.global [%0], [%1], 16;" ::"r"(dst), "l"(src) : "memory"); }
__device__ __forceinline__ void cp_async_commit() { asm volatile("cp.async.commit_group;" ::: "memory"); }
template <int N>
__device__ __forceinline__ void cp_async_wait() { asm volatile("cp.async.wait_group %0;" ::"n"(N) : "memory"); }
__device__ __forceinline__ void mbar_init(uint32_t bar, uint32_t count) { asm volatile("mbarrier.init.shared::cta.b64 [%0], %1;" ::"r"(bar), "r"(count) : "memory"); }
__device__ __forceinline__ void mbar_arrive(uint32_t bar) { asm volatile("mbarrier.arrive.shared::cta.b64 _, [%0];" ::"r"(bar) : "memory"); }
__device__ __forceinline__ void mbar_wait(uint32_t bar, uint32_t parity) {
  asm volatile(
      "{\n .reg .pred p;\n"
      "WAIT:\n mbarrier.try_wait.parity.shared::cta.b64 p, [%0], %1;\n"
      " @!p bra WAIT;\n}" ::"r"(bar), "r"(parity) : "memory");
}
template <int ID, int N>
__device__ __forceinline__ void named_bar_sync() { asm volatile("bar.sync %0, %1;" ::"n"(ID), "n"(N) : "memory"); }
template <int R>
__device__ __forceinline__ void setmaxnreg_dec() { asm volatile("setmaxnreg.dec.sync.aligned.u32 %0;" ::"n"(R)); }
template <int R>
__device__ __forceinline__ void setmaxnreg_inc() { asm volatile("setmaxnreg.inc.sync.aligned.u32 %0;" ::"n"(R)); }
__device__ __forceinline__ void wgmma_tf32(float (&d)[128], uint64_t a_desc, uint64_t b_desc) {
  asm volatile(
      "wgmma.mma_async.sync.aligned.m64n256k8.f32.tf32.tf32 {"
      "%0, %1, %2, %3, %4, %5, %6, %7, %8, %9, %10, %11, %12, %13, %14, %15, "
      "%16, %17, %18, %19, %20, %21, %22, %23, %24, %25, %26, %27, %28, %29, %30, %31, "
      "%32, %33, %34, %35, %36, %37, %38, %39, %40, %41, %42, %43, %44, %45, %46, %47, "
      "%48, %49, %50, %51, %52, %53, %54, %55, %56, %57, %58, %59, %60, %61, %62, %63, "
      "%64, %65, %66, %67, %68, %69, %70, %71, %72, %73, %74, %75, %76, %77, %78, %79, "
      "%80, %81, %82, %83, %84, %85, %86, %87, %88, %89, %90, %91, %92, %93, %94, %95, "
      "%96, %97, %98, %99, %100, %101, %102, %103, %104, %105, %106, %107, %108, %109, %110, %111, "
      "%112, %113, %114, %115, %116, %117, %118, %119, %120, %121, %122, %123, %124, %125, %126, %127 "
      "}, %128, %129, 1, 1, 1;"
      : "+f"(d[0]), "+f"(d[1]), "+f"(d[2]), "+f"(d[3]), "+f"(d[4]), "+f"(d[5]), "+f"(d[6]), "+f"(d[7]),
        "+f"(d[8]), "+f"(d[9]), "+f"(d[10]), "+f"(d[11]), "+f"(d[12]), "+f"(d[13]), "+f"(d[14]), "+f"(d[15]),
        "+f"(d[16]), "+f"(d[17]), "+f"(d[18]), "+f"(d[19]), "+f"(d[20]), "+f"(d[21]), "+f"(d[22]), "+f"(d[23]),
        "+f"(d[24]), "+f"(d[25]), "+f"(d[26]), "+f"(d[27]), "+f"(d[28]), "+f"(d[29]), "+f"(d[30]), "+f"(d[31]),
        "+f"(d[32]), "+f"(d[33]), "+f"(d[34]), "+f"(d[35]), "+f"(d[36]), "+f"(d[37]), "+f"(d[38]), "+f"(d[39]),
        "+f"(d[40]), "+f"(d[41]), "+f"(d[42]), "+f"(d[43]), "+f"(d[44]), "+f"(d[45]), "+f"(d[46]), "+f"(d[47]),
        "+f"(d[48]), "+f"(d[49]), "+f"(d[50]), "+f"(d[51]), "+f"(d[52]), "+f"(d[53]), "+f"(d[54]), "+f"(d[55]),
        "+f"(d[56]), "+f"(d[57]), "+f"(d[58]), "+f"(d[59]), "+f"(d[60]), "+f"(d[61]), "+f"(d[62]), "+f"(d[63]),
        "+f"(d[64]), "+f"(d[65]), "+f"(d[66]), "+f"(d[67]), "+f"(d[68]), "+f"(d[69]), "+f"(d[70]), "+f"(d[71]),
        "+f"(d[72]), "+f"(d[73]), "+f"(d[74]), "+f"(d[75]), "+f"(d[76]), "+f"(d[77]), "+f"(d[78]), "+f"(d[79]),
        "+f"(d[80]), "+f"(d[81]), "+f"(d[82]), "+f"(d[83]), "+f"(d[84]), "+f"(d[85]), "+f"(d[86]), "+f"(d[87]),
        "+f"(d[88]), "+f"(d[89]), "+f"(d[90]), "+f"(d[91]), "+f"(d[92]), "+f"(d[93]), "+f"(d[94]), "+f"(d[95]),
        "+f"(d[96]), "+f"(d[97]), "+f"(d[98]), "+f"(d[99]), "+f"(d[100]), "+f"(d[101]), "+f"(d[102]), "+f"(d[103]),
        "+f"(d[104]), "+f"(d[105]), "+f"(d[106]), "+f"(d[107]), "+f"(d[108]), "+f"(d[109]), "+f"(d[110]), "+f"(d[111]),
        "+f"(d[112]), "+f"(d[113]), "+f"(d[114]), "+f"(d[115]), "+f"(d[116]), "+f"(d[117]), "+f"(d[118]), "+f"(d[119]),
        "+f"(d[120]), "+f"(d[121]), "+f"(d[122]), "+f"(d[123]), "+f"(d[124]), "+f"(d[125]), "+f"(d[126]), "+f"(d[127])
      : "l"(a_desc), "l"(b_desc));
}
__device__ __forceinline__ uint64_t make_desc(uint32_t smem_addr) {
  return (uint64_t)((smem_addr >> 4) & 0x3FFF) | ((uint64_t)1 << 16) | ((uint64_t)(512 >> 4) << 32) | ((uint64_t)2 << 62);
}
__device__ __forceinline__ uint32_t sw64(int r, int c) { return (uint32_t)((r >> 3) * 512 + (r & 7) * 64 + ((c ^ ((r >> 1) & 3)) << 4)); }
__device__ __forceinline__ void sts128(uint32_t addr, uint32_t x, uint32_t y, uint32_t z, uint32_t w) {
  asm volatile("st.shared.v4.b32 [%0], {%1, %2, %3, %4};" ::"r"(addr), "r"(x), "r"(y), "r"(z), "r"(w) : "memory");
}
__device__ __forceinline__ uint4 lds128(uint32_t addr) {
  uint4 v;
  asm volatile("ld.shared.v4.b32 {%0, %1, %2, %3}, [%4];" : "=r"(v.x), "=r"(v.y), "=r"(v.z), "=r"(v.w) : "r"(addr));
  return v;
}
__device__ __forceinline__ uint32_t hi_of(uint32_t x) { return x & 0xFFFFE000u; }
__device__ __forceinline__ uint32_t lo_of(uint32_t x) { return __float_as_uint(__uint_as_float(x) - __uint_as_float(x & 0xFFFFE000u)); }
__device__ __forceinline__ void store_chunk(uint32_t hi_tile, uint32_t lo_tile, uint32_t off, uint4 v, bool split) {
  sts128(hi_tile + off, hi_of(v.x), hi_of(v.y), hi_of(v.z), hi_of(v.w));
  if (split) sts128(lo_tile + off, lo_of(v.x), lo_of(v.y), lo_of(v.z), lo_of(v.w));
}
__device__ __forceinline__ void store_block_t(uint32_t hi_tile, uint32_t lo_tile, int c4, int kg, const uint4 (&v)[4], bool split) {
  uint4 q0 = make_uint4(v[0].x, v[1].x, v[2].x, v[3].x), q1 = make_uint4(v[0].y, v[1].y, v[2].y, v[3].y);
  uint4 q2 = make_uint4(v[0].z, v[1].z, v[2].z, v[3].z), q3 = make_uint4(v[0].w, v[1].w, v[2].w, v[3].w);
  const int s = (c4 >> 1) & 3;
  if (s & 1) { const uint4 t = q0; q0 = q1; q1 = q2; q2 = q3; q3 = t; }
  if (s & 2) { uint4 t = q0; q0 = q2; q2 = t; t = q1; q1 = q3; q3 = t; }
  store_chunk(hi_tile, lo_tile, sw64(4 * c4 + (s & 3), kg), q0, split);
  store_chunk(hi_tile, lo_tile, sw64(4 * c4 + ((s + 1) & 3), kg), q1, split);
  store_chunk(hi_tile, lo_tile, sw64(4 * c4 + ((s + 2) & 3), kg), q2, split);
  store_chunk(hi_tile, lo_tile, sw64(4 * c4 + ((s + 3) & 3), kg), q3, split);
}

struct TcParams {
  GemmArgs g;
  int tiles_m;
  int split;
  const float* head_w;
  const float* head_b;
  float* head_out;
  int64_t head_gs, head_out_gs;
  int head_n, store_c;
  int head_js, head_ns;
  TcFuseL1 l1;
};

template <int EPI, bool FUSE = false>
__global__ void __launch_bounds__(THREADS, 1) tc_gemm_kernel(const TcParams p) {
  extern __shared__ uint8_t smem_raw[];
  uint8_t* smem = reinterpret_cast<uint8_t*>((reinterpret_cast<uintptr_t>(smem_raw) + BAR_BYTES + 511) & ~(uintptr_t)511);
  float* head_s = reinterpret_cast<float*>(smem + head_off(FUSE));
  const uint32_t stage0 = smem_u32(smem), raw0 = stage0 + RAW_OFF;
  const uint32_t full0 = stage0 - BAR_BYTES, empty0 = full0 + N_STAGES * 8;
  const uint32_t w1s = stage0 + l1_off(FUSE), b1s = w1s + L1_W_BYTES, xs = b1s + L1_B_BYTES;
  constexpr uint32_t RAW_A = 0, RAW_B = raw_a_bytes(FUSE), RAW_BYTES = raw_bytes(FUSE);

  const int tid = threadIdx.x, warp = tid >> 5, lane = tid & 31, wg = tid >> 7;
  const GemmArgs& g = p.g;
  const int nkb = g.K / BK, tiles_m = p.tiles_m;
  const int my_tiles = (g.G * tiles_m - (int)blockIdx.x + (int)gridDim.x - 1) / (int)gridDim.x;
  const int nq = my_tiles * nkb;
  auto tile_of = [&](int i) { return (int)blockIdx.x + i * (int)gridDim.x; };

  if (tid == 0) {
#pragma unroll
    for (int s = 0; s < N_STAGES; ++s) {
      mbar_init(full0 + 8 * s, PRODUCER_THREADS);
      mbar_init(empty0 + 8 * s, CONSUMER_THREADS);
    }
  }
  __syncthreads();

  if (wg == 0) {
    setmaxnreg_dec<producer_regs(FUSE)>();
    const bool a_km = FUSE || g.a_kmajor != 0, b_km = g.b_kmajor != 0, split = p.split != 0;
    constexpr int MAP = 2 * PRODUCER_THREADS;
    const int pt = tid;

    auto copy_kb = [&](int q) {
      if (q < nq) {
        const int t = tile_of(q / nkb), kb = q % nkb, grp = t / tiles_m, m0 = (t % tiles_m) * BM;
        const float* A = g.A + (int64_t)(grp / g.a_gdiv) * g.a_gs;
        const float* Bg = g.B + (int64_t)(grp / g.b_gdiv) * g.b_gs;
#pragma unroll
        for (int h = 0; h < 2; ++h) {
          const int v = pt + h * PRODUCER_THREADS, fr = v >> 2, fc = v & 3;
          const uint32_t raw = raw0 + (uint32_t)(q % RAW_STAGES) * RAW_BYTES + (uint32_t)v * 16u;
          if (!FUSE) {
            if (a_km) {
              const float* src = A + (int64_t)(m0 + fr) * g.lda + kb * BK + fc * 4;
              cp_async16(raw + RAW_A, src);
              cp_async16(raw + RAW_A + MAP * 16, src + (int64_t)64 * g.lda);
            } else if (h == 0) {
              const float* src = A + (int64_t)(kb * BK + ((v >> 5) & 3) * 4) * g.lda + m0 + (v & 31) * 4;
#pragma unroll
              for (int k = 0; k < 4; ++k) cp_async16(raw + RAW_A + k * (MAP / 2) * 16, src + (int64_t)k * g.lda);
            }
          }
          const float* src = b_km ? Bg + (int64_t)fr * g.ldb + kb * BK + fc * 4 : Bg + (int64_t)(kb * BK + (v >> 6) * 4) * g.ldb + (v & 63) * 4;
          const int64_t step = b_km ? (int64_t)64 * g.ldb : (int64_t)g.ldb;
#pragma unroll
          for (int j = 0; j < 4; ++j) cp_async16(raw + RAW_B + j * MAP * 16, src + j * step);
        }
      }
      cp_async_commit();
    };

    auto split_kb = [&](int q, int s) {
      const uint32_t st = stage0 + (uint32_t)s * STAGE_BYTES;
#pragma unroll(FUSE ? 1 : 2)
      for (int h = 0; h < 2; ++h) {
        const int v = pt + h * PRODUCER_THREADS, fr = v >> 2, fc = v & 3;
        const uint32_t raw = raw0 + (uint32_t)(q % RAW_STAGES) * RAW_BYTES + (uint32_t)v * 16u;
        const uint32_t km_off = sw64(fr, fc);
        if (FUSE) {
          const int kb = q % nkb, k0 = kb * BK + fc * 4;
          const uint4 bq = lds128(b1s + (uint32_t)k0 * 4u);
          float c0[4] = {__uint_as_float(bq.x), __uint_as_float(bq.y), __uint_as_float(bq.z), __uint_as_float(bq.w)};
          float c1[4] = {c0[0], c0[1], c0[2], c0[3]};
          const int np = (p.l1.x_k + 3) >> 2;
#pragma unroll
          for (int c4 = 0; c4 < L1_MAXK / 4; ++c4) {
            if (c4 < np) {
              const uint4 x0 = lds128(xs + sw64(fr, c4)), x1 = lds128(xs + sw64(fr + 64, c4));
#pragma unroll
              for (int qq = 0; qq < 4; ++qq) {
                const uint4 w = lds128(w1s + (uint32_t)((k0 + qq) * 64 + ((c4 ^ fc) << 4)));
                c0[qq] = fmaf(__uint_as_float(x0.x), __uint_as_float(w.x), c0[qq]); c1[qq] = fmaf(__uint_as_float(x1.x), __uint_as_float(w.x), c1[qq]);
                c0[qq] = fmaf(__uint_as_float(x0.y), __uint_as_float(w.y), c0[qq]); c1[qq] = fmaf(__uint_as_float(x1.y), __uint_as_float(w.y), c1[qq]);
                c0[qq] = fmaf(__uint_as_float(x0.z), __uint_as_float(w.z), c0[qq]); c1[qq] = fmaf(__uint_as_float(x1.z), __uint_as_float(w.z), c1[qq]);
                c0[qq] = fmaf(__uint_as_float(x0.w), __uint_as_float(w.w), c0[qq]); c1[qq] = fmaf(__uint_as_float(x1.w), __uint_as_float(w.w), c1[qq]);
              }
            }
          }
          const uint4 a0 = make_uint4(__float_as_uint(fmaxf(c0[0], 0.f)), __float_as_uint(fmaxf(c0[1], 0.f)), __float_as_uint(fmaxf(c0[2], 0.f)), __float_as_uint(fmaxf(c0[3], 0.f)));
          const uint4 a1 = make_uint4(__float_as_uint(fmaxf(c1[0], 0.f)), __float_as_uint(fmaxf(c1[1], 0.f)), __float_as_uint(fmaxf(c1[2], 0.f)), __float_as_uint(fmaxf(c1[3], 0.f)));
          store_chunk(st + A_HI, st + A_LO, km_off, a0, split);
          store_chunk(st + A_HI, st + A_LO, km_off + 4096u, a1, split);
          if (p.l1.store) {
            const int t = tile_of(q / nkb);
            float* hs = p.l1.store + (int64_t)(t / tiles_m) * p.l1.store_gs + (int64_t)((t % tiles_m) * BM + fr) * g.K + k0;
            *reinterpret_cast<uint4*>(hs) = a0;
            *reinterpret_cast<uint4*>(hs + (int64_t)64 * g.K) = a1;
          }
        } else if (a_km) {
          store_chunk(st + A_HI, st + A_LO, km_off, lds128(raw + RAW_A), split);
          store_chunk(st + A_HI, st + A_LO, km_off + 4096u, lds128(raw + RAW_A + MAP * 16), split);
        } else if (h == 0) {
          uint4 va[4];
#pragma unroll
          for (int k = 0; k < 4; ++k) va[k] = lds128(raw + RAW_A + k * (MAP / 2) * 16);
          store_block_t(st + A_HI, st + A_LO, v & 31, (v >> 5) & 3, va, split);
        }
        if (b_km) {
#pragma unroll
          for (int j = 0; j < 4; ++j) store_chunk(st + B_HI, st + B_LO, km_off + (uint32_t)j * 4096u, lds128(raw + RAW_B + j * MAP * 16), split);
        } else {
          uint4 vb[4];
#pragma unroll
          for (int k = 0; k < 4; ++k) vb[k] = lds128(raw + RAW_B + k * MAP * 16);
          store_block_t(st + B_HI, st + B_LO, v & 63, v >> 6, vb, split);
        }
      }
    };

    auto stage_l1 = [&](int t) {
      const int grp = t / tiles_m, m0 = (t % tiles_m) * BM, xk = p.l1.x_k;
      const float* w1 = p.l1.w1 + (int64_t)grp * p.l1.gs;
      const float* b1 = p.l1.b1 + (int64_t)grp * p.l1.gs;
      const float* x = p.l1.x + (int64_t)(grp / p.l1.x_gdiv) * p.l1.x_gs + (int64_t)m0 * p.l1.x_ld;
      float* w1f = reinterpret_cast<float*>(smem + l1_off(FUSE));
      float* b1f = reinterpret_cast<float*>(smem + l1_off(FUSE) + L1_W_BYTES);
      float* xf = reinterpret_cast<float*>(smem + l1_off(FUSE) + L1_W_BYTES + L1_B_BYTES);
#pragma unroll 1
      for (int i = pt; i < L1_ROWS * L1_MAXK; i += PRODUCER_THREADS) {
        const int k = i / L1_MAXK, j = i % L1_MAXK;
        w1f[k * L1_MAXK + ((((j >> 2) ^ ((k >> 2) & 3)) << 2) | (j & 3))] = (k < g.K && j < xk) ? __ldg(w1 + (int64_t)k * xk + j) : 0.f;
      }
      for (int i = pt; i < L1_ROWS; i += PRODUCER_THREADS) b1f[i] = i < g.K ? __ldg(b1 + i) : 0.f;
#pragma unroll 1
      for (int i = pt; i < BM * L1_MAXK; i += PRODUCER_THREADS) {
        const int r = i / L1_MAXK, j = i % L1_MAXK;
        xf[(sw64(r, j >> 2) >> 2) + (j & 3)] = j < xk ? __ldg(x + (int64_t)r * p.l1.x_ld + j) : 0.f;
      }
    };

#pragma unroll 1
    for (int q = 0; q < RAW_STAGES; ++q) copy_kb(q);
    int s = 0;
    uint32_t ph = 1;
#pragma unroll 1
    for (int q = 0; q < nq; ++q) {
      if (FUSE && q % nkb == 0) {
        if (q > 0) named_bar_sync<PRODUCER_BAR, PRODUCER_THREADS>();
        stage_l1(tile_of(q / nkb));
        named_bar_sync<PRODUCER_BAR, PRODUCER_THREADS>();
      }
      mbar_wait(empty0 + 8 * s, ph);
      cp_async_wait<RAW_STAGES - 1>();
      split_kb(q, s);
      fence_proxy_async();
      mbar_arrive(full0 + 8 * s);
      copy_kb(q + RAW_STAGES);
      if (++s == N_STAGES) { s = 0; ph ^= 1; }
    }
    cp_async_wait<0>();
    return;
  }

  setmaxnreg_inc<consumer_regs(FUSE)>();
  const int cw = wg - 1, ct = tid - PRODUCER_THREADS;
  const uint64_t a_desc0 = make_desc(stage0 + (uint32_t)cw * 4096u), b_desc0 = make_desc(stage0);
  const bool split = p.split != 0;
  float acc[128];
  int s = 0;
  uint32_t ph = 0;
#pragma unroll 1
  for (int i = 0; i < my_tiles; ++i) {
#pragma unroll
    for (int j = 0; j < 128; ++j) acc[j] = 0.f;
    int prev = 0;
#pragma unroll 1
    for (int kb = 0; kb < nkb; ++kb) {
      mbar_wait(full0 + 8 * s, ph);
      const uint32_t cur = (uint32_t)s * STAGE_BYTES;
      wgmma_fence();
#pragma unroll
      for (int kk = 0; kk < BK / 8; ++kk) {
        const uint32_t o = cur + kk * 32;
        const uint64_t ah = a_desc0 + ((o + A_HI) >> 4), al = a_desc0 + ((o + A_LO) >> 4), bh = b_desc0 + ((o + B_HI) >> 4), bl = b_desc0 + ((o + B_LO) >> 4);
        if (split) {
          wgmma_tf32(acc, al, bh);
          wgmma_tf32(acc, ah, bl);
        }
        wgmma_tf32(acc, ah, bh);
      }
      wgmma_commit();
      wgmma_wait<1>();
      if (kb > 0) mbar_arrive(empty0 + 8 * prev);
      prev = s;
      if (++s == N_STAGES) { s = 0; ph ^= 1; }
    }

    const int t = tile_of(i), grp = t / tiles_m, m0 = (t % tiles_m) * BM;
    if (EPI == 4 || EPI == 6) {
      named_bar_sync<CONSUMER_BAR, CONSUMER_THREADS>();
      const float* wsrc = p.head_w + (int64_t)grp * p.head_gs;
      if (EPI == 4) head_s[ct] = __ldg(g.bias + (int64_t)grp * g.bias_gs + ct);
#pragma unroll
      for (int j = 0; j < HEAD_MAX; ++j)
        if (j < p.head_n) head_s[BN + j * BN + ct] = __ldg(wsrc + (int64_t)j * p.head_js + (int64_t)ct * p.head_ns);
    }
    wgmma_wait<0>();
    mbar_arrive(empty0 + 8 * prev);
    if (EPI == 4 || EPI == 6) named_bar_sync<CONSUMER_BAR, CONSUMER_THREADS>();
    const int r0 = m0 + cw * 64 + (warp & 3) * 16 + (lane >> 2), cl = (lane & 3) * 2;
    float* C = g.C + (int64_t)grp * g.c_gs + (int64_t)r0 * g.ldc + cl;
    const int64_t c8 = (int64_t)8 * g.ldc;
    const float* bias = (EPI == 1 || (EPI == 3 && g.bias)) ? g.bias + (int64_t)grp * g.bias_gs + cl : nullptr;
    const float* mask = (EPI == 2 || (EPI == 3 && g.mask)) ? g.mask + (int64_t)grp * g.mask_gs + (int64_t)r0 * g.ldmask + cl : nullptr;
    const int64_t m8 = (int64_t)8 * g.ldmask;
    const uint32_t* mbits = (EPI == 5 || EPI == 6) ? g.mask_bits + (int64_t)grp * g.mask_bits_gs + (int64_t)r0 * (BN / 32) : nullptr;
    uint32_t word0 = 0, word1 = 0;
#pragma unroll
    for (int c = 0; c < BN / 8; ++c) {
      float v00 = acc[4 * c], v01 = acc[4 * c + 1], v10 = acc[4 * c + 2], v11 = acc[4 * c + 3];
      const int col = 8 * c, bit = (c & 3) * 8 + cl;
      if (EPI == 5 || EPI == 6) {
        if ((c & 3) == 0) { word0 = __ldg(mbits + (c >> 2)); word1 = __ldg(mbits + 8 * (BN / 32) + (c >> 2)); }
        v00 = (word0 >> bit) & 1u ? v00 : 0.f; v01 = (word0 >> (bit + 1)) & 1u ? v01 : 0.f;
        v10 = (word1 >> bit) & 1u ? v10 : 0.f; v11 = (word1 >> (bit + 1)) & 1u ? v11 : 0.f;
      }
      if (EPI == 4) {
        const float2 b = *reinterpret_cast<const float2*>(head_s + col + cl);
        v00 = fmaxf(v00 + b.x, 0.f); v01 = fmaxf(v01 + b.y, 0.f); v10 = fmaxf(v10 + b.x, 0.f); v11 = fmaxf(v11 + b.y, 0.f);
        if (g.bits_out) {
          if ((c & 3) == 0) word0 = word1 = 0;
          word0 |= (v00 > 0.f ? 1u : 0u) << bit | (v01 > 0.f ? 1u : 0u) << (bit + 1);
          word1 |= (v10 > 0.f ? 1u : 0u) << bit | (v11 > 0.f ? 1u : 0u) << (bit + 1);
          if ((c & 3) == 3) {
            word0 |= __shfl_xor_sync(0xffffffffu, word0, 1); word0 |= __shfl_xor_sync(0xffffffffu, word0, 2);
            word1 |= __shfl_xor_sync(0xffffffffu, word1, 1); word1 |= __shfl_xor_sync(0xffffffffu, word1, 2);
            if ((lane & 3) == 0) {
              uint32_t* bo = g.bits_out + (int64_t)grp * g.bits_out_gs + (int64_t)r0 * (BN / 32) + (c >> 2);
              bo[0] = word0;
              bo[8 * (BN / 32)] = word1;
            }
          }
        }
      }
      if (EPI == 4 || EPI == 6) {
        acc[4 * c] = v00; acc[4 * c + 1] = v01; acc[4 * c + 2] = v10; acc[4 * c + 3] = v11;
        if (!p.store_c) continue;
      }
      if (EPI == 1) {
        const float2 b = __ldg(reinterpret_cast<const float2*>(bias + col));
        v00 = fmaxf(v00 + b.x, 0.f); v01 = fmaxf(v01 + b.y, 0.f); v10 = fmaxf(v10 + b.x, 0.f); v11 = fmaxf(v11 + b.y, 0.f);
      } else if (EPI == 2) {
        const float2 ma = __ldg(reinterpret_cast<const float2*>(mask + col)), mb = __ldg(reinterpret_cast<const float2*>(mask + m8 + col));
        v00 = ma.x > 0.f ? v00 : 0.f; v01 = ma.y > 0.f ? v01 : 0.f; v10 = mb.x > 0.f ? v10 : 0.f; v11 = mb.y > 0.f ? v11 : 0.f;
      } else if (EPI == 3) {
        if (bias) {
          const float2 b = __ldg(reinterpret_cast<const float2*>(bias + col));
          v00 += b.x; v01 += b.y; v10 += b.x; v11 += b.y;
        }
        if (g.act >= 0) { v00 = act_apply(v00, g.act); v01 = act_apply(v01, g.act); v10 = act_apply(v10, g.act); v11 = act_apply(v11, g.act); }
        if (mask) {
          const float2 ma = __ldg(reinterpret_cast<const float2*>(mask + col)), mb = __ldg(reinterpret_cast<const float2*>(mask + m8 + col));
          v00 *= act_grad_from_output(ma.x, g.mask_act); v01 *= act_grad_from_output(ma.y, g.mask_act);
          v10 *= act_grad_from_output(mb.x, g.mask_act); v11 *= act_grad_from_output(mb.y, g.mask_act);
        }
      }
      *reinterpret_cast<float2*>(C + col) = make_float2(v00, v01);
      *reinterpret_cast<float2*>(C + c8 + col) = make_float2(v10, v11);
    }
    if (EPI == 4 || EPI == 6) {
      float* ho = p.head_out + (int64_t)grp * p.head_out_gs + (int64_t)r0 * p.head_n;
      const float* hb = p.head_b ? p.head_b + (int64_t)grp * p.head_gs : nullptr;
#pragma unroll 1
      for (int j = 0; j < HEAD_MAX; ++j) {
        if (j < p.head_n) {
          float s0 = 0.f, s1 = 0.f;
#pragma unroll
          for (int c = 0; c < BN / 8; ++c) {
            const float2 w = *reinterpret_cast<const float2*>(head_s + BN + j * BN + 8 * c + cl);
            s0 = fmaf(acc[4 * c], w.x, s0); s0 = fmaf(acc[4 * c + 1], w.y, s0);
            s1 = fmaf(acc[4 * c + 2], w.x, s1); s1 = fmaf(acc[4 * c + 3], w.y, s1);
          }
          s0 += __shfl_xor_sync(0xffffffffu, s0, 1); s0 += __shfl_xor_sync(0xffffffffu, s0, 2);
          s1 += __shfl_xor_sync(0xffffffffu, s1, 1); s1 += __shfl_xor_sync(0xffffffffu, s1, 2);
          if ((lane & 3) == 0) {
            const float b = hb ? __ldg(hb + j) : 0.f;
            ho[j] = s0 + b;
            ho[(int64_t)8 * p.head_n + j] = s1 + b;
          }
        }
      }
    }
  }
}


__global__ void colsum_kernel(const float* __restrict__ A, int64_t a_gs, int a_gdiv, int lda, int K, int M, float* __restrict__ out, int64_t out_gs) {
  const int g = blockIdx.y, m = blockIdx.x * blockDim.x + threadIdx.x;
  if (m >= M) return;
  const float* a = A + (int64_t)(g / a_gdiv) * a_gs + m;
  float s = 0.f;
  for (int k = 0; k < K; ++k) s += a[(int64_t)k * lda];
  out[(int64_t)g * out_gs + m] = s;
}

}

bool tc_gemm_eligible(const GemmArgs& a) {
  auto al16 = [](const void* p) { return (reinterpret_cast<uintptr_t>(p) & 15) == 0; };
  if (a.M % BM != 0 || a.N != BN || a.K % BK != 0 || a.accumulate) return false;
  if (a.a_kmajor == 0 && a.b_kmajor != 0) return false;
  if (!al16(a.A) || !al16(a.B) || !al16(a.C) || a.lda % 4 || a.ldb % 4 || a.ldc % 4 || a.a_gs % 4 || a.b_gs % 4 || a.c_gs % 4) return false;
  if (a.bias && (!al16(a.bias) || a.bias_gs % 4)) return false;
  if (a.mask && (!al16(a.mask) || a.ldmask % 4 || a.mask_gs % 4)) return false;
  return true;
}

template <int EPI, bool FUSE = false>
int tc_set_attr() {
  IL_CUDA(cudaFuncSetAttribute(tc_gemm_kernel<EPI, FUSE>, cudaFuncAttributeMaxDynamicSharedMemorySize, smem_bytes(FUSE)));
  return 0;
}

int tc_gemm_init() {
  IL_TRY((tc_set_attr<0>())); IL_TRY((tc_set_attr<1>())); IL_TRY((tc_set_attr<2>())); IL_TRY((tc_set_attr<3>())); IL_TRY((tc_set_attr<4>()));
  IL_TRY((tc_set_attr<4, true>())); IL_TRY((tc_set_attr<5>())); IL_TRY((tc_set_attr<6>()));
  return 0;
}

template <int EPI, bool FUSE = false>
static int tc_launch(il_handle* h, TcParams& p, cudaStream_t stream) {
  const GemmArgs& a = p.g;
  p.tiles_m = a.M / BM;
  const int tiles = a.G * p.tiles_m, wave = h->sm_count >= p.tiles_m ? h->sm_count / p.tiles_m * p.tiles_m : h->sm_count;
  IL_LAUNCH(h, (tc_gemm_kernel<EPI, FUSE>), tiles < wave ? tiles : wave, THREADS, smem_bytes(FUSE), stream, p);
  return 0;
}

bool tc_head_fusable(const il_handle* h, const GemmArgs& a, int head_n) {
  return h->gemm_mode != IL_GEMM_FP32 && tc_gemm_eligible(a) && a.bias && a.act == IL_ACT_RELU && !a.mask && !a.colsum && head_n >= 1 && head_n <= HEAD_MAX;
}

bool tc_l1_fusable(const il_handle* h, const GemmArgs& a, int x_k) {
  return h->tc_fuse_l1 && tc_gemm_eligible(a) && x_k >= 1 && x_k <= L1_MAXK && a.K <= L1_ROWS && a.a_kmajor;
}

int launch_tc_gemm_head(il_handle* h, const GemmArgs& a, const float* head_w, const float* head_b, int64_t head_gs, int head_n, float* head_out, int64_t head_out_gs, int store_c,
                        cudaStream_t stream, const TcFuseL1* l1) {
  IL_CHECK(tc_head_fusable(h, a, head_n), "tc_gemm_head: not fusable");
  TcParams p{};
  p.g = a;
  p.split = h->gemm_mode == IL_GEMM_TF32X3 ? 1 : 0;
  p.head_w = head_w; p.head_b = head_b; p.head_out = head_out; p.head_gs = head_gs; p.head_out_gs = head_out_gs; p.head_n = head_n; p.store_c = store_c;
  p.head_js = BN; p.head_ns = 1;
  double bytes = gemm_algorithmic_bytes(a, store_c != 0) + 4.0 * a.G * (double)a.M * head_n, flops = 2.0 * a.M * a.N * a.K * a.G;
  if (l1) {
    IL_CHECK(tc_l1_fusable(h, a, l1->x_k), "tc_gemm_head: first layer not fusable (K0=%d)", l1->x_k);
    IL_CHECK(l1->x && l1->w1 && l1->b1 && (reinterpret_cast<uintptr_t>(l1->b1) & 15) == 0 && l1->gs % 4 == 0, "tc_gemm_head: bad first-layer buffers");
    IL_CHECK(!l1->store || ((reinterpret_cast<uintptr_t>(l1->store) & 15) == 0 && l1->store_gs % 4 == 0), "tc_gemm_head: unaligned hidden store");
    p.l1 = *l1;
    const double gx = (a.G + l1->x_gdiv - 1) / l1->x_gdiv;
    bytes += -4.0 * a.G * (double)a.M * a.K + 4.0 * (gx * a.M * l1->x_k + (double)a.G * a.K * (l1->x_k + 1)) + (l1->store ? 4.0 * a.G * (double)a.M * a.K : 0.0);
    flops += 2.0 * a.G * (double)a.M * a.K * l1->x_k;
  }
  auto run = [&]() { return l1 ? tc_launch<4, true>(h, p, stream) : tc_launch<4>(h, p, stream); };
  if (h->profiling) {
    ProfiledLaunch pl;
    IL_TRY(profile_open(h, &pl, flops, bytes, stream));
    const int rc = run();
    IL_TRY(profile_close(h, &pl, stream));
    return rc;
  }
  return run();
}

bool tc_dx_head_fusable(const il_handle* h, const GemmArgs& a, int head_n) {
  return h->gemm_mode != IL_GEMM_FP32 && a.M >= 128 && a.K >= 128 && tc_gemm_eligible(a) && a.mask_bits && !a.mask && !a.bias && a.act < 0 && !a.colsum && a.mask_act == IL_ACT_RELU &&
         head_n >= 1 && head_n <= HEAD_MAX;
}
int launch_tc_gemm_dx_head(il_handle* h, const GemmArgs& a, const float* w, int64_t w_gs, int w_ns, int head_n, float* out, int64_t out_gs, cudaStream_t stream) {
  IL_CHECK(tc_dx_head_fusable(h, a, head_n), "tc_gemm_dx_head: not fusable");
  TcParams p{};
  p.g = a;
  p.split = h->gemm_mode == IL_GEMM_TF32X3 ? 1 : 0;
  p.head_w = w; p.head_b = nullptr; p.head_out = out; p.head_gs = w_gs; p.head_out_gs = out_gs; p.head_n = head_n; p.store_c = 0;
  p.head_js = 1; p.head_ns = w_ns;
  const double bytes = gemm_algorithmic_bytes(a, false) + 4.0 * a.G * (double)a.M * head_n, flops = 2.0 * a.M * a.N * a.K * a.G;
  if (h->profiling) {
    ProfiledLaunch pl;
    IL_TRY(profile_open(h, &pl, flops, bytes, stream));
    const int rc = tc_launch<6>(h, p, stream);
    IL_TRY(profile_close(h, &pl, stream));
    return rc;
  }
  return tc_launch<6>(h, p, stream);
}

int launch_tc_gemm(il_handle* h, const GemmArgs& a, cudaStream_t stream) {
  IL_CHECK(tc_gemm_eligible(a), "tc_gemm: shape/layout not eligible (M=%d N=%d K=%d)", a.M, a.N, a.K);
  TcParams p{};
  p.g = a;
  p.split = h->gemm_mode == IL_GEMM_TF32X3 ? 1 : 0;
  const bool bits = a.mask_bits != nullptr;
  IL_CHECK(!bits || (!a.bias && a.act < 0 && a.mask_act == IL_ACT_RELU), "tc_gemm: sign-bit masks are the ReLU derivative of a plain product");
  if (bits) p.g.mask = nullptr;
  const bool plain = !a.bias && a.act < 0 && !a.mask && !bits;
  const bool bias_relu = a.bias && a.act == IL_ACT_RELU && !a.mask;
  const bool mask_relu = !a.bias && a.act < 0 && a.mask && a.mask_act == IL_ACT_RELU && !bits;
  if (bits) IL_TRY(tc_launch<5>(h, p, stream));
  else if (plain) IL_TRY(tc_launch<0>(h, p, stream));
  else if (bias_relu) IL_TRY(tc_launch<1>(h, p, stream));
  else if (mask_relu) IL_TRY(tc_launch<2>(h, p, stream));
  else IL_TRY(tc_launch<3>(h, p, stream));
  if (a.colsum) {
    dim3 cg((a.M + 127) / 128, a.G);
    IL_LAUNCH(h, colsum_kernel, cg, 128, 0, stream, a.A, a.a_gs, a.a_gdiv, a.lda, a.K, a.M, a.colsum, a.colsum_gs);
  }
  return 0;
}
```

Measured before the change: 82520.

## Compute first layer in registers and feed wgmma A fragments directly, enabled by default

The fused first-layer path now computes the layer-1 hidden activations in consumer registers and passes them to wgmma as register-sourced A operands, instead of staging the A tile in shared memory. The first-layer weights, bias and input are double-buffered through dedicated mbarriers, and the kernel is specialised on the input width. ReLU sign bits for layers 0 and 1 are emitted from the fused kernel so hidden activations need not be stored. The fusion becomes on by default. The change adds register pressure and shared memory use in the consumer warps, and the fused path is limited to a few input widths and a hidden size of exactly 256.

```diff
diff --git a/imitation-learning_b200/csrc/api.cu b/imitation-learning_b200/csrc/api.cu
--- a/imitation-learning_b200/csrc/api.cu
+++ b/imitation-learning_b200/csrc/api.cu
@@ -45,7 +45,7 @@
     const char* gt = getenv("IL_GAIL_TILED");
     h->gail_tiled = (gt && gt[0] == '0') ? 0 : 1;
     const char* fl = getenv("IL_TC_FUSE_L1");
-    h->tc_fuse_l1 = (fl && fl[0] == '1') ? 1 : 0;
+    h->tc_fuse_l1 = (fl && fl[0] == '0') ? 0 : 1;
     const char* th = getenv("IL_THIN_HOIST");
     h->thin_hoist = (th && th[0] == '0') ? 0 : 1;
   }
diff --git a/imitation-learning_b200/csrc/common.cuh b/imitation-learning_b200/csrc/common.cuh
--- a/imitation-learning_b200/csrc/common.cuh
+++ b/imitation-learning_b200/csrc/common.cuh
@@ -204,6 +204,8 @@
   int64_t gs;
   float* store;
   int64_t store_gs;
+  uint32_t* bits;
+  int64_t bits_gs;
 };
 bool tc_head_fusable(const il_handle* h, const GemmArgs& a, int head_n);
 bool tc_l1_fusable(const il_handle* h, const GemmArgs& a, int x_k);
diff --git a/imitation-learning_b200/csrc/mlp.cu b/imitation-learning_b200/csrc/mlp.cu
--- a/imitation-learning_b200/csrc/mlp.cu
+++ b/imitation-learning_b200/csrc/mlp.cu
@@ -86,12 +86,16 @@
     if (head_shape && l == 0 && L == 3) {
       GemmArgs a1 = layer_args(1);
       a1.A = nullptr; a1.a_gs = 0; a1.a_gdiv = 1; a1.lda = m->dims[1];
-      if (tc_head_fusable(h, a1, m->dims[L]) && tc_l1_fusable(h, a1, m->dims[0])) {
+      if (tc_head_fusable(h, a1, m->dims[L]) && tc_l1_fusable(h, a1, m->dims[0]) && gemm_first_layer_emits_bits(h, layer_args(0))) {
         TcFuseL1 f{};
         f.x = X.ptr; f.x_gs = X.gs; f.x_gdiv = X.gdiv; f.x_ld = X.ld; f.x_k = m->dims[0];
         f.w1 = m->params + o.w[0]; f.b1 = m->params + o.b[0]; f.gs = m->stride;
-        f.store = keep_hidden ? acts.hid[0] : nullptr; f.store_gs = (int64_t)n * m->dims[1];
-        IL_TRY(launch_tc_gemm_head(h, a1, m->params + o.w[L - 1], m->params + o.b[L - 1], m->stride, m->dims[L], out, out_gs, keep_hidden ? 1 : 0, stream, &f));
+        const bool bits0 = want_bits && acts.bits[0];
+        const bool bits1 = want_bits && keep == MLP_KEEP_MASKS && acts.bits[1] && m->dims[L] <= HB_MAXN;
+        if (bits0) { f.bits = acts.bits[0]; f.bits_gs = (int64_t)n * (m->dims[1] / 32); acts.bits_valid[0] = true; }
+        if (bits1) { a1.bits_out = acts.bits[1]; a1.bits_out_gs = (int64_t)n * (m->dims[2] / 32); acts.bits_valid[1] = true; }
+        f.store = keep == MLP_KEEP_ALL || (keep_hidden && !bits0) ? acts.hid[0] : nullptr; f.store_gs = (int64_t)n * m->dims[1];
+        IL_TRY(launch_tc_gemm_head(h, a1, m->params + o.w[L - 1], m->params + o.b[L - 1], m->stride, m->dims[L], out, out_gs, keep_hidden && !bits1 ? 1 : 0, stream, &f));
         return 0;
       }
     }
diff --git a/imitation-learning_b200/csrc/tc_gemm.cu b/imitation-learning_b200/csrc/tc_gemm.cu
--- a/imitation-learning_b200/csrc/tc_gemm.cu
+++ b/imitation-learning_b200/csrc/tc_gemm.cu
@@ -7,28 +7,30 @@
 constexpr int BM = 128, BN = 256, BK = 16;
 constexpr int PRODUCER_THREADS = 128, CONSUMER_THREADS = 256;
 constexpr int THREADS = PRODUCER_THREADS + CONSUMER_THREADS;
-constexpr int LAUNCH_REGS = 168;
-constexpr int producer_regs(bool fuse) { return fuse ? 72 : 56; }
-constexpr int consumer_regs(bool fuse) { return (THREADS * LAUNCH_REGS - PRODUCER_THREADS * producer_regs(fuse)) / CONSUMER_THREADS; }
-static_assert(THREADS * LAUNCH_REGS <= 65536 && consumer_regs(false) % 8 == 0 && consumer_regs(true) % 8 == 0, "tc_gemm: setmaxnreg split");
-constexpr int CONSUMER_BAR = 1, PRODUCER_BAR = 2;
+constexpr int LAUNCH_REGS = 168, PRODUCER_REGS = 56;
+constexpr int CONSUMER_REGS = (THREADS * LAUNCH_REGS - PRODUCER_THREADS * PRODUCER_REGS) / CONSUMER_THREADS;
+static_assert(THREADS * LAUNCH_REGS <= 65536 && CONSUMER_REGS % 8 == 0, "tc_gemm: setmaxnreg split");
+constexpr int CONSUMER_BAR = 1;
 constexpr int A_BYTES = BM * BK * 4, B_BYTES = BN * BK * 4;
-constexpr int A_HI = 0, A_LO = A_BYTES, B_HI = 2 * A_BYTES, B_LO = 2 * A_BYTES + B_BYTES;
-constexpr int STAGE_BYTES = 2 * (A_BYTES + B_BYTES);
 constexpr int N_STAGES = 3;
 constexpr int RAW_STAGES = 3;
 constexpr int HEAD_MAX = 8;
 constexpr int HEAD_BYTES = (BN + HEAD_MAX * BN) * 4;
 constexpr int L1_MAXK = 16, L1_ROWS = 256;
 constexpr int L1_W_BYTES = L1_ROWS * L1_MAXK * 4, L1_B_BYTES = L1_ROWS * 4, L1_X_BYTES = BM * L1_MAXK * 4;
-constexpr int raw_a_bytes(bool fuse) { return fuse ? 0 : A_BYTES; }
-constexpr int raw_bytes(bool fuse) { return raw_a_bytes(fuse) + B_BYTES; }
-constexpr int RAW_OFF = N_STAGES * STAGE_BYTES;
-constexpr int head_off(bool fuse) { return RAW_OFF + RAW_STAGES * raw_bytes(fuse); }
+constexpr int L1_BUF_BYTES = L1_W_BYTES + L1_B_BYTES + L1_X_BYTES;
+constexpr int a_bytes(bool fuse) { return fuse ? 0 : A_BYTES; }
+constexpr int A_HI = 0, A_LO = A_BYTES;
+constexpr int b_hi(bool fuse) { return 2 * a_bytes(fuse); }
+constexpr int b_lo(bool fuse) { return 2 * a_bytes(fuse) + B_BYTES; }
+constexpr int stage_bytes(bool fuse) { return 2 * (a_bytes(fuse) + B_BYTES); }
+constexpr int raw_bytes(bool fuse) { return a_bytes(fuse) + B_BYTES; }
+constexpr int raw_off(bool fuse) { return N_STAGES * stage_bytes(fuse); }
+constexpr int head_off(bool fuse) { return raw_off(fuse) + RAW_STAGES * raw_bytes(fuse); }
 constexpr int l1_off(bool fuse) { return head_off(fuse) + HEAD_BYTES; }
-constexpr int BAR_BYTES = 64;
-static_assert(2 * N_STAGES * 8 <= BAR_BYTES && BAR_BYTES + 512 - 16 <= 1024, "tc_gemm: mbarrier area");
-constexpr int smem_bytes(bool fuse) { return 1024 + l1_off(fuse) + (fuse ? L1_W_BYTES + L1_B_BYTES + L1_X_BYTES : 0); }
+constexpr int BAR_BYTES = 128;
+static_assert(2 * N_STAGES * 8 + 4 * 8 <= BAR_BYTES && BAR_BYTES + 512 - 16 <= 1024, "tc_gemm: mbarrier area");
+constexpr int smem_bytes(bool fuse) { return 1024 + l1_off(fuse) + (fuse ? 2 * L1_BUF_BYTES : 0); }
 static_assert(smem_bytes(false) <= 227 * 1024 && smem_bytes(true) <= 227 * 1024, "tc_gemm: shared memory over the 227 KB per-CTA limit");
 
 __device__ __forceinline__ uint32_t smem_u32(const void* p) { return (uint32_t)__cvta_generic_to_shared(p); }
@@ -38,6 +40,9 @@
 template <int N>
 __device__ __forceinline__ void wgmma_wait() { asm volatile("wgmma.wait_group.sync.aligned %0;" ::"n"(N) : "memory"); }
 __device__ __forceinline__ void cp_async16(uint32_t dst, const float* src) { asm volatile("cp.async.cg.shared.global [%0], [%1], 16;" ::"r"(dst), "l"(src) : "memory"); }
+__device__ __forceinline__ void cp_async4(uint32_t dst, const float* src, bool valid) {
+  asm volatile("cp.async.ca.shared.global [%0], [%1], 4, %2;" ::"r"(dst), "l"(src), "r"(valid ? 4 : 0) : "memory");
+}
 __device__ __forceinline__ void cp_async_commit() { asm volatile("cp.async.commit_group;" ::: "memory"); }
 template <int N>
 __device__ __forceinline__ void cp_async_wait() { asm volatile("cp.async.wait_group %0;" ::"n"(N) : "memory"); }
@@ -55,46 +60,64 @@
 __device__ __forceinline__ void setmaxnreg_dec() { asm volatile("setmaxnreg.dec.sync.aligned.u32 %0;" ::"n"(R)); }
 template <int R>
 __device__ __forceinline__ void setmaxnreg_inc() { asm volatile("setmaxnreg.inc.sync.aligned.u32 %0;" ::"n"(R)); }
+#define IL_WGMMA_D                                                                                                                 \
+  "{%0, %1, %2, %3, %4, %5, %6, %7, %8, %9, %10, %11, %12, %13, %14, %15, "                                                        \
+  "%16, %17, %18, %19, %20, %21, %22, %23, %24, %25, %26, %27, %28, %29, %30, %31, "                                               \
+  "%32, %33, %34, %35, %36, %37, %38, %39, %40, %41, %42, %43, %44, %45, %46, %47, "                                               \
+  "%48, %49, %50, %51, %52, %53, %54, %55, %56, %57, %58, %59, %60, %61, %62, %63, "                                               \
+  "%64, %65, %66, %67, %68, %69, %70, %71, %72, %73, %74, %75, %76, %77, %78, %79, "                                               \
+  "%80, %81, %82, %83, %84, %85, %86, %87, %88, %89, %90, %91, %92, %93, %94, %95, "                                               \
+  "%96, %97, %98, %99, %100, %101, %102, %103, %104, %105, %106, %107, %108, %109, %110, %111, "                                    \
+  "%112, %113, %114, %115, %116, %117, %118, %119, %120, %121, %122, %123, %124, %125, %126, %127}"
+#define IL_WGMMA_D_OPERANDS(d)                                                                                                      \
+  "+f"(d[0]), "+f"(d[1]), "+f"(d[2]), "+f"(d[3]), "+f"(d[4]), "+f"(d[5]), "+f"(d[6]), "+f"(d[7]),                                   \
+  "+f"(d[8]), "+f"(d[9]), "+f"(d[10]), "+f"(d[11]), "+f"(d[12]), "+f"(d[13]), "+f"(d[14]), "+f"(d[15]),                             \
+  "+f"(d[16]), "+f"(d[17]), "+f"(d[18]), "+f"(d[19]), "+f"(d[20]), "+f"(d[21]), "+f"(d[22]), "+f"(d[23]),                           \
+  "+f"(d[24]), "+f"(d[25]), "+f"(d[26]), "+f"(d[27]), "+f"(d[28]), "+f"(d[29]), "+f"(d[30]), "+f"(d[31]),                           \
+  "+f"(d[32]), "+f"(d[33]), "+f"(d[34]), "+f"(d[35]), "+f"(d[36]), "+f"(d[37]), "+f"(d[38]), "+f"(d[39]),                           \
+  "+f"(d[40]), "+f"(d[41]), "+f"(d[42]), "+f"(d[43]), "+f"(d[44]), "+f"(d[45]), "+f"(d[46]), "+f"(d[47]),                           \
+  "+f"(d[48]), "+f"(d[49]), "+f"(d[50]), "+f"(d[51]), "+f"(d[52]), "+f"(d[53]), "+f"(d[54]), "+f"(d[55]),                           \
+  "+f"(d[56]), "+f"(d[57]), "+f"(d[58]), "+f"(d[59]), "+f"(d[60]), "+f"(d[61]), "+f"(d[62]), "+f"(d[63]),                           \
+  "+f"(d[64]), "+f"(d[65]), "+f"(d[66]), "+f"(d[67]), "+f"(d[68]), "+f"(d[69]), "+f"(d[70]), "+f"(d[71]),                           \
+  "+f"(d[72]), "+f"(d[73]), "+f"(d[74]), "+f"(d[75]), "+f"(d[76]), "+f"(d[77]), "+f"(d[78]), "+f"(d[79]),                           \
+  "+f"(d[80]), "+f"(d[81]), "+f"(d[82]), "+f"(d[83]), "+f"(d[84]), "+f"(d[85]), "+f"(d[86]), "+f"(d[87]),                           \
+  "+f"(d[88]), "+f"(d[89]), "+f"(d[90]), "+f"(d[91]), "+f"(d[92]), "+f"(d[93]), "+f"(d[94]), "+f"(d[95]),                           \
+  "+f"(d[96]), "+f"(d[97]), "+f"(d[98]), "+f"(d[99]), "+f"(d[100]), "+f"(d[101]), "+f"(d[102]), "+f"(d[103]),                       \
+  "+f"(d[104]), "+f"(d[105]), "+f"(d[106]), "+f"(d[107]), "+f"(d[108]), "+f"(d[109]), "+f"(d[110]), "+f"(d[111]),                   \
+  "+f"(d[112]), "+f"(d[113]), "+f"(d[114]), "+f"(d[115]), "+f"(d[116]), "+f"(d[117]), "+f"(d[118]), "+f"(d[119]),                   \
+  "+f"(d[120]), "+f"(d[121]), "+f"(d[122]), "+f"(d[123]), "+f"(d[124]), "+f"(d[125]), "+f"(d[126]), "+f"(d[127])
 __device__ __forceinline__ void wgmma_tf32(float (&d)[128], uint64_t a_desc, uint64_t b_desc) {
-  asm volatile(
-      "wgmma.mma_async.sync.aligned.m64n256k8.f32.tf32.tf32 {"
-      "%0, %1, %2, %3, %4, %5, %6, %7, %8, %9, %10, %11, %12, %13, %14, %15, "
-      "%16, %17, %18, %19, %20, %21, %22, %23, %24, %25, %26, %27, %28, %29, %30, %31, "
-      "%32, %33, %34, %35, %36, %37, %38, %39, %40, %41, %42, %43, %44, %45, %46, %47, "
-      "%48, %49, %50, %51, %52, %53, %54, %55, %56, %57, %58, %59, %60, %61, %62, %63, "
-      "%64, %65, %66, %67, %68, %69, %70, %71, %72, %73, %74, %75, %76, %77, %78, %79, "
-      "%80, %81, %82, %83, %84, %85, %86, %87, %88, %89, %90, %91, %92, %93, %94, %95, "
-      "%96, %97, %98, %99, %100, %101, %102, %103, %104, %105, %106, %107, %108, %109, %110, %111, "
-      "%112, %113, %114, %115, %116, %117, %118, %119, %120, %121, %122, %123, %124, %125, %126, %127 "
-      "}, %128, %129, 1, 1, 1;"
-      : "+f"(d[0]), "+f"(d[1]), "+f"(d[2]), "+f"(d[3]), "+f"(d[4]), "+f"(d[5]), "+f"(d[6]), "+f"(d[7]),
-        "+f"(d[8]), "+f"(d[9]), "+f"(d[10]), "+f"(d[11]), "+f"(d[12]), "+f"(d[13]), "+f"(d[14]), "+f"(d[15]),
-        "+f"(d[16]), "+f"(d[17]), "+f"(d[18]), "+f"(d[19]), "+f"(d[20]), "+f"(d[21]), "+f"(d[22]), "+f"(d[23]),
-        "+f"(d[24]), "+f"(d[25]), "+f"(d[26]), "+f"(d[27]), "+f"(d[28]), "+f"(d[29]), "+f"(d[30]), "+f"(d[31]),
-        "+f"(d[32]), "+f"(d[33]), "+f"(d[34]), "+f"(d[35]), "+f"(d[36]), "+f"(d[37]), "+f"(d[38]), "+f"(d[39]),
-        "+f"(d[40]), "+f"(d[41]), "+f"(d[42]), "+f"(d[43]), "+f"(d[44]), "+f"(d[45]), "+f"(d[46]), "+f"(d[47]),
-        "+f"(d[48]), "+f"(d[49]), "+f"(d[50]), "+f"(d[51]), "+f"(d[52]), "+f"(d[53]), "+f"(d[54]), "+f"(d[55]),
-        "+f"(d[56]), "+f"(d[57]), "+f"(d[58]), "+f"(d[59]), "+f"(d[60]), "+f"(d[61]), "+f"(d[62]), "+f"(d[63]),
-        "+f"(d[64]), "+f"(d[65]), "+f"(d[66]), "+f"(d[67]), "+f"(d[68]), "+f"(d[69]), "+f"(d[70]), "+f"(d[71]),
-        "+f"(d[72]), "+f"(d[73]), "+f"(d[74]), "+f"(d[75]), "+f"(d[76]), "+f"(d[77]), "+f"(d[78]), "+f"(d[79]),
-        "+f"(d[80]), "+f"(d[81]), "+f"(d[82]), "+f"(d[83]), "+f"(d[84]), "+f"(d[85]), "+f"(d[86]), "+f"(d[87]),
-        "+f"(d[88]), "+f"(d[89]), "+f"(d[90]), "+f"(d[91]), "+f"(d[92]), "+f"(d[93]), "+f"(d[94]), "+f"(d[95]),
-        "+f"(d[96]), "+f"(d[97]), "+f"(d[98]), "+f"(d[99]), "+f"(d[100]), "+f"(d[101]), "+f"(d[102]), "+f"(d[103]),
-        "+f"(d[104]), "+f"(d[105]), "+f"(d[106]), "+f"(d[107]), "+f"(d[108]), "+f"(d[109]), "+f"(d[110]), "+f"(d[111]),
-        "+f"(d[112]), "+f"(d[113]), "+f"(d[114]), "+f"(d[115]), "+f"(d[116]), "+f"(d[117]), "+f"(d[118]), "+f"(d[119]),
-        "+f"(d[120]), "+f"(d[121]), "+f"(d[122]), "+f"(d[123]), "+f"(d[124]), "+f"(d[125]), "+f"(d[126]), "+f"(d[127])
-      : "l"(a_desc), "l"(b_desc));
+  asm volatile("wgmma.mma_async.sync.aligned.m64n256k8.f32.tf32.tf32 " IL_WGMMA_D ", %128, %129, 1, 1, 1;"
+               : IL_WGMMA_D_OPERANDS(d)
+               : "l"(a_desc), "l"(b_desc));
+}
+__device__ __forceinline__ void wgmma_tf32_ra(float (&d)[128], const uint32_t (&a)[4], uint64_t b_desc) {
+  asm volatile("wgmma.mma_async.sync.aligned.m64n256k8.f32.tf32.tf32 " IL_WGMMA_D ", {%128, %129, %130, %131}, %132, 1, 1, 1;"
+               : IL_WGMMA_D_OPERANDS(d)
+               : "r"(a[0]), "r"(a[1]), "r"(a[2]), "r"(a[3]), "l"(b_desc));
+}
+__device__ __forceinline__ void fence_frags(uint32_t (&h)[2][4], uint32_t (&l)[2][4]) {
+#pragma unroll
+  for (int kk = 0; kk < 2; ++kk)
+#pragma unroll
+    for (int u = 0; u < 4; ++u) asm volatile("" : "+r"(h[kk][u]), "+r"(l[kk][u])::"memory");
 }
 __device__ __forceinline__ uint64_t make_desc(uint32_t smem_addr) {
   return (uint64_t)((smem_addr >> 4) & 0x3FFF) | ((uint64_t)1 << 16) | ((uint64_t)(512 >> 4) << 32) | ((uint64_t)2 << 62);
 }
 __device__ __forceinline__ uint32_t sw64(int r, int c) { return (uint32_t)((r >> 3) * 512 + (r & 7) * 64 + ((c ^ ((r >> 1) & 3)) << 4)); }
+__device__ __forceinline__ uint32_t l1_w_off(int n, int j) { return (uint32_t)(n * 64 + ((((j >> 2) ^ (n & 3)) << 4) | ((j & 3) << 2))); }
 __device__ __forceinline__ void sts128(uint32_t addr, uint32_t x, uint32_t y, uint32_t z, uint32_t w) {
   asm volatile("st.shared.v4.b32 [%0], {%1, %2, %3, %4};" ::"r"(addr), "r"(x), "r"(y), "r"(z), "r"(w) : "memory");
 }
 __device__ __forceinline__ uint4 lds128(uint32_t addr) {
   uint4 v;
   asm volatile("ld.shared.v4.b32 {%0, %1, %2, %3}, [%4];" : "=r"(v.x), "=r"(v.y), "=r"(v.z), "=r"(v.w) : "r"(addr));
+  return v;
+}
+__device__ __forceinline__ float lds32(uint32_t addr) {
+  float v;
+  asm volatile("ld.shared.f32 %0, [%1];" : "=f"(v) : "r"(addr));
   return v;
 }
 __device__ __forceinline__ uint32_t hi_of(uint32_t x) { return x & 0xFFFFE000u; }
@@ -128,15 +151,17 @@
   TcFuseL1 l1;
 };
 
-template <int EPI, bool FUSE = false>
+template <int EPI, int L1K = 0>
 __global__ void __launch_bounds__(THREADS, 1) tc_gemm_kernel(const TcParams p) {
+  constexpr bool FUSE = L1K > 0;
   extern __shared__ uint8_t smem_raw[];
   uint8_t* smem = reinterpret_cast<uint8_t*>((reinterpret_cast<uintptr_t>(smem_raw) + BAR_BYTES + 511) & ~(uintptr_t)511);
   float* head_s = reinterpret_cast<float*>(smem + head_off(FUSE));
-  const uint32_t stage0 = smem_u32(smem), raw0 = stage0 + RAW_OFF;
+  const uint32_t stage0 = smem_u32(smem), raw0 = stage0 + raw_off(FUSE);
   const uint32_t full0 = stage0 - BAR_BYTES, empty0 = full0 + N_STAGES * 8;
-  const uint32_t w1s = stage0 + l1_off(FUSE), b1s = w1s + L1_W_BYTES, xs = b1s + L1_B_BYTES;
-  constexpr uint32_t RAW_A = 0, RAW_B = raw_a_bytes(FUSE), RAW_BYTES = raw_bytes(FUSE);
+  const uint32_t l1_full0 = empty0 + N_STAGES * 8, l1_empty0 = l1_full0 + 16;
+  const uint32_t l1s0 = stage0 + l1_off(FUSE);
+  constexpr uint32_t STAGE_BYTES = stage_bytes(FUSE), RAW_BYTES = raw_bytes(FUSE), RAW_A = 0, RAW_B = a_bytes(FUSE), B_HI = b_hi(FUSE), B_LO = b_lo(FUSE);
 
   const int tid = threadIdx.x, warp = tid >> 5, lane = tid & 31, wg = tid >> 7;
   const GemmArgs& g = p.g;
@@ -151,18 +176,45 @@
       mbar_init(full0 + 8 * s, PRODUCER_THREADS);
       mbar_init(empty0 + 8 * s, CONSUMER_THREADS);
     }
+    if (FUSE) {
+#pragma unroll
+      for (int u = 0; u < 2; ++u) {
+        mbar_init(l1_full0 + 8 * u, PRODUCER_THREADS);
+        mbar_init(l1_empty0 + 8 * u, CONSUMER_THREADS);
+      }
+    }
   }
   __syncthreads();
 
   if (wg == 0) {
-    setmaxnreg_dec<producer_regs(FUSE)>();
-    const bool a_km = FUSE || g.a_kmajor != 0, b_km = g.b_kmajor != 0, split = p.split != 0;
+    setmaxnreg_dec<PRODUCER_REGS>();
+    const bool a_km = g.a_kmajor != 0, b_km = g.b_kmajor != 0, split = p.split != 0;
     constexpr int MAP = 2 * PRODUCER_THREADS;
     const int pt = tid;
+
+    auto stage_l1 = [&](int i) {
+      mbar_wait(l1_empty0 + 8 * (i & 1), ((i >> 1) & 1) ^ 1);
+      const int t = tile_of(i), grp = t / tiles_m, m0 = (t % tiles_m) * BM, xk = L1K;
+      const float* w1 = p.l1.w1 + (int64_t)grp * p.l1.gs;
+      const float* x = p.l1.x + (int64_t)(grp / p.l1.x_gdiv) * p.l1.x_gs + (int64_t)m0 * p.l1.x_ld;
+      const uint32_t buf = l1s0 + (uint32_t)(i & 1) * L1_BUF_BYTES;
+#pragma unroll 1
+      for (int e = pt; e < L1_ROWS * L1_MAXK; e += PRODUCER_THREADS) {
+        const int n = e / L1_MAXK, j = e % L1_MAXK;
+        cp_async4(buf + l1_w_off(n, j), w1 + (j < xk ? n * xk + j : 0), j < xk);
+      }
+#pragma unroll 1
+      for (int e = pt; e < BM * L1_MAXK; e += PRODUCER_THREADS) {
+        const int r = e / L1_MAXK, j = e % L1_MAXK;
+        cp_async4(buf + L1_W_BYTES + L1_B_BYTES + sw64(r, j >> 2) + (j & 3) * 4, x + (j < xk ? (int64_t)r * p.l1.x_ld + j : 0), j < xk);
+      }
+      if (pt < L1_ROWS / 4) cp_async16(buf + L1_W_BYTES + pt * 16, p.l1.b1 + (int64_t)grp * p.l1.gs + 4 * pt);
+    };
 
     auto copy_kb = [&](int q) {
       if (q < nq) {
         const int t = tile_of(q / nkb), kb = q % nkb, grp = t / tiles_m, m0 = (t % tiles_m) * BM;
+        if (FUSE && kb == 0) stage_l1(q / nkb);
         const float* A = g.A + (int64_t)(grp / g.a_gdiv) * g.a_gs;
         const float* Bg = g.B + (int64_t)(grp / g.b_gdiv) * g.b_gs;
 #pragma unroll
@@ -191,49 +243,21 @@
 
     auto split_kb = [&](int q, int s) {
       const uint32_t st = stage0 + (uint32_t)s * STAGE_BYTES;
-#pragma unroll(FUSE ? 1 : 2)
+#pragma unroll
       for (int h = 0; h < 2; ++h) {
         const int v = pt + h * PRODUCER_THREADS, fr = v >> 2, fc = v & 3;
         const uint32_t raw = raw0 + (uint32_t)(q % RAW_STAGES) * RAW_BYTES + (uint32_t)v * 16u;
         const uint32_t km_off = sw64(fr, fc);
-        if (FUSE) {
-          const int kb = q % nkb, k0 = kb * BK + fc * 4;
-          const uint4 bq = lds128(b1s + (uint32_t)k0 * 4u);
-          float c0[4] = {__uint_as_float(bq.x), __uint_as_float(bq.y), __uint_as_float(bq.z), __uint_as_float(bq.w)};
-          float c1[4] = {c0[0], c0[1], c0[2], c0[3]};
-          const int np = (p.l1.x_k + 3) >> 2;
-#pragma unroll
-          for (int c4 = 0; c4 < L1_MAXK / 4; ++c4) {
-            if (c4 < np) {
-              const uint4 x0 = lds128(xs + sw64(fr, c4)), x1 = lds128(xs + sw64(fr + 64, c4));
-#pragma unroll
-              for (int qq = 0; qq < 4; ++qq) {
-                const uint4 w = lds128(w1s + (uint32_t)((k0 + qq) * 64 + ((c4 ^ fc) << 4)));
-                c0[qq] = fmaf(__uint_as_float(x0.x), __uint_as_float(w.x), c0[qq]); c1[qq] = fmaf(__uint_as_float(x1.x), __uint_as_float(w.x), c1[qq]);
-                c0[qq] = fmaf(__uint_as_float(x0.y), __uint_as_float(w.y), c0[qq]); c1[qq] = fmaf(__uint_as_float(x1.y), __uint_as_float(w.y), c1[qq]);
-                c0[qq] = fmaf(__uint_as_float(x0.z), __uint_as_float(w.z), c0[qq]); c1[qq] = fmaf(__uint_as_float(x1.z), __uint_as_float(w.z), c1[qq]);
-                c0[qq] = fmaf(__uint_as_float(x0.w), __uint_as_float(w.w), c0[qq]); c1[qq] = fmaf(__uint_as_float(x1.w), __uint_as_float(w.w), c1[qq]);
-              }
-            }
+        if (!FUSE) {
+          if (a_km) {
+            store_chunk(st + A_HI, st + A_LO, km_off, lds128(raw + RAW_A), split);
+            store_chunk(st + A_HI, st + A_LO, km_off + 4096u, lds128(raw + RAW_A + MAP * 16), split);
+          } else if (h == 0) {
+            uint4 va[4];
+#pragma unroll
+            for (int k = 0; k < 4; ++k) va[k] = lds128(raw + RAW_A + k * (MAP / 2) * 16);
+            store_block_t(st + A_HI, st + A_LO, v & 31, (v >> 5) & 3, va, split);
           }
-          const uint4 a0 = make_uint4(__float_as_uint(fmaxf(c0[0], 0.f)), __float_as_uint(fmaxf(c0[1], 0.f)), __float_as_uint(fmaxf(c0[2], 0.f)), __float_as_uint(fmaxf(c0[3], 0.f)));
-          const uint4 a1 = make_uint4(__float_as_uint(fmaxf(c1[0], 0.f)), __float_as_uint(fmaxf(c1[1], 0.f)), __float_as_uint(fmaxf(c1[2], 0.f)), __float_as_uint(fmaxf(c1[3], 0.f)));
-          store_chunk(st + A_HI, st + A_LO, km_off, a0, split);
-          store_chunk(st + A_HI, st + A_LO, km_off + 4096u, a1, split);
-          if (p.l1.store) {
-            const int t = tile_of(q / nkb);
-            float* hs = p.l1.store + (int64_t)(t / tiles_m) * p.l1.store_gs + (int64_t)((t % tiles_m) * BM + fr) * g.K + k0;
-            *reinterpret_cast<uint4*>(hs) = a0;
-            *reinterpret_cast<uint4*>(hs + (int64_t)64 * g.K) = a1;
-          }
-        } else if (a_km) {
-          store_chunk(st + A_HI, st + A_LO, km_off, lds128(raw + RAW_A), split);
-          store_chunk(st + A_HI, st + A_LO, km_off + 4096u, lds128(raw + RAW_A + MAP * 16), split);
-        } else if (h == 0) {
-          uint4 va[4];
-#pragma unroll
-          for (int k = 0; k < 4; ++k) va[k] = lds128(raw + RAW_A + k * (MAP / 2) * 16);
-          store_block_t(st + A_HI, st + A_LO, v & 31, (v >> 5) & 3, va, split);
         }
         if (b_km) {
 #pragma unroll
@@ -247,40 +271,15 @@
       }
     };
 
-    auto stage_l1 = [&](int t) {
-      const int grp = t / tiles_m, m0 = (t % tiles_m) * BM, xk = p.l1.x_k;
-      const float* w1 = p.l1.w1 + (int64_t)grp * p.l1.gs;
-      const float* b1 = p.l1.b1 + (int64_t)grp * p.l1.gs;
-      const float* x = p.l1.x + (int64_t)(grp / p.l1.x_gdiv) * p.l1.x_gs + (int64_t)m0 * p.l1.x_ld;
-      float* w1f = reinterpret_cast<float*>(smem + l1_off(FUSE));
-      float* b1f = reinterpret_cast<float*>(smem + l1_off(FUSE) + L1_W_BYTES);
-      float* xf = reinterpret_cast<float*>(smem + l1_off(FUSE) + L1_W_BYTES + L1_B_BYTES);
-#pragma unroll 1
-      for (int i = pt; i < L1_ROWS * L1_MAXK; i += PRODUCER_THREADS) {
-        const int k = i / L1_MAXK, j = i % L1_MAXK;
-        w1f[k * L1_MAXK + ((((j >> 2) ^ ((k >> 2) & 3)) << 2) | (j & 3))] = (k < g.K && j < xk) ? __ldg(w1 + (int64_t)k * xk + j) : 0.f;
-      }
-      for (int i = pt; i < L1_ROWS; i += PRODUCER_THREADS) b1f[i] = i < g.K ? __ldg(b1 + i) : 0.f;
-#pragma unroll 1
-      for (int i = pt; i < BM * L1_MAXK; i += PRODUCER_THREADS) {
-        const int r = i / L1_MAXK, j = i % L1_MAXK;
-        xf[(sw64(r, j >> 2) >> 2) + (j & 3)] = j < xk ? __ldg(x + (int64_t)r * p.l1.x_ld + j) : 0.f;
-      }
-    };
-
 #pragma unroll 1
     for (int q = 0; q < RAW_STAGES; ++q) copy_kb(q);
     int s = 0;
     uint32_t ph = 1;
 #pragma unroll 1
     for (int q = 0; q < nq; ++q) {
-      if (FUSE && q % nkb == 0) {
-        if (q > 0) named_bar_sync<PRODUCER_BAR, PRODUCER_THREADS>();
-        stage_l1(tile_of(q / nkb));
-        named_bar_sync<PRODUCER_BAR, PRODUCER_THREADS>();
-      }
       mbar_wait(empty0 + 8 * s, ph);
       cp_async_wait<RAW_STAGES - 1>();
+      if (FUSE && q % nkb == 0) mbar_arrive(l1_full0 + 8 * ((q / nkb) & 1));
       split_kb(q, s);
       fence_proxy_async();
       mbar_arrive(full0 + 8 * s);
@@ -291,38 +290,165 @@
     return;
   }
 
-  setmaxnreg_inc<consumer_regs(FUSE)>();
+  setmaxnreg_inc<CONSUMER_REGS>();
   const int cw = wg - 1, ct = tid - PRODUCER_THREADS;
   const uint64_t a_desc0 = make_desc(stage0 + (uint32_t)cw * 4096u), b_desc0 = make_desc(stage0);
   const bool split = p.split != 0;
   float acc[128];
   int s = 0;
   uint32_t ph = 0;
+  const int lr = cw * 64 + (warp & 3) * 16 + (lane >> 2), qt = lane & 3;
+
+  uint32_t wbits0 = 0, wbits1 = 0;
+  uint32_t keep0[2] = {0, 0}, keep1[2] = {0, 0};
+  auto l1_frag = [&](int kb, uint32_t l1b, float* hs, uint32_t (&fh)[2][4], uint32_t (&fl)[2][4]) {
+    constexpr int xk = L1K, npf = xk >> 1;
+    constexpr bool odd = (xk & 1) != 0;
+    const uint32_t wrow = l1b + (uint32_t)(16 * kb + qt) * 64u, xrow = l1b + L1_W_BYTES + L1_B_BYTES;
+    const uint32_t brow = l1b + L1_W_BYTES + (uint32_t)(16 * kb + qt) * 4u;
+    float e[2][4], o[2][4];
+#pragma unroll
+    for (int c = 0; c < L1_MAXK / 4; ++c) {
+      if (4 * c < xk) {
+        const uint4 x0 = lds128(xrow + sw64(lr, c)), x1 = lds128(xrow + sw64(lr + 8, c));
+        const float xv[2][4] = {{__uint_as_float(x0.x), __uint_as_float(x0.y), __uint_as_float(x0.z), __uint_as_float(x0.w)},
+                                {__uint_as_float(x1.x), __uint_as_float(x1.y), __uint_as_float(x1.z), __uint_as_float(x1.w)}};
+#pragma unroll
+        for (int j = 0; j < 4; ++j) {
+          const uint4 wq = lds128(wrow + (uint32_t)j * 256u + (uint32_t)((c ^ qt) << 4));
+          const float wv[4] = {__uint_as_float(wq.x), __uint_as_float(wq.y), __uint_as_float(wq.z), __uint_as_float(wq.w)};
+#pragma unroll
+          for (int hh = 0; hh < 2; ++hh) {
+            const int kp = 2 * c + hh;
+#pragma unroll
+            for (int r = 0; r < 2; ++r) {
+              const float xe = xv[r][2 * hh], xo = xv[r][2 * hh + 1], we = wv[2 * hh], wo = wv[2 * hh + 1];
+              if (kp == 0) {
+                e[r][j] = odd ? __fmul_rn(xe, we) : fmaf(xe, we, lds32(brow + 16u * j));
+                o[r][j] = odd ? __fmul_rn(xo, wo) : fmaf(xo, wo, 0.f);
+              } else if (kp < npf) {
+                e[r][j] = fmaf(xe, we, e[r][j]);
+                o[r][j] = fmaf(xo, wo, o[r][j]);
+              } else if (odd && kp == npf) {
+                e[r][j] = fmaf(xe, we, e[r][j]);
+                o[r][j] = fmaf(1.f, lds32(brow + 16u * j), o[r][j]);
+              }
+            }
+          }
+        }
+      }
+    }
+    float v[2][4];
+#pragma unroll
+    for (int r = 0; r < 2; ++r)
+#pragma unroll
+      for (int j = 0; j < 4; ++j) v[r][j] = fmaxf(e[r][j] + o[r][j], 0.f);
+#pragma unroll
+    for (int kk = 0; kk < 2; ++kk) {
+      const uint32_t a[4] = {__float_as_uint(v[0][2 * kk]), __float_as_uint(v[1][2 * kk]), __float_as_uint(v[0][2 * kk + 1]), __float_as_uint(v[1][2 * kk + 1])};
+#pragma unroll
+      for (int u = 0; u < 4; ++u) { fh[kk][u] = hi_of(a[u]); fl[kk][u] = lo_of(a[u]); }
+    }
+    if (p.l1.bits) {
+      const int sh = 16 * (kb & 1) + qt;
+#pragma unroll
+      for (int j = 0; j < 4; ++j) { wbits0 |= (v[0][j] > 0.f ? 1u : 0u) << (sh + 4 * j); wbits1 |= (v[1][j] > 0.f ? 1u : 0u) << (sh + 4 * j); }
+      if (kb & 1) {
+        wbits0 |= __shfl_xor_sync(0xffffffffu, wbits0, 1); wbits0 |= __shfl_xor_sync(0xffffffffu, wbits0, 2);
+        wbits1 |= __shfl_xor_sync(0xffffffffu, wbits1, 1); wbits1 |= __shfl_xor_sync(0xffffffffu, wbits1, 2);
+        if ((kb >> 2) == qt) {
+          if ((kb >> 1) & 1) { keep0[1] = wbits0; keep1[1] = wbits1; }
+          else { keep0[0] = wbits0; keep1[0] = wbits1; }
+        }
+        wbits0 = wbits1 = 0;
+      }
+    }
+    if (hs) {
+#pragma unroll
+      for (int r = 0; r < 2; ++r) {
+        float* w = v[r];
+        const bool b0 = qt & 1, b1 = (qt >> 1) & 1;
+        float r0 = __shfl_xor_sync(0xffffffffu, b0 ? w[0] : w[1], 1), r1 = __shfl_xor_sync(0xffffffffu, b0 ? w[2] : w[3], 1);
+        if (b0) { w[0] = r0; w[2] = r1; } else { w[1] = r0; w[3] = r1; }
+        r0 = __shfl_xor_sync(0xffffffffu, b1 ? w[0] : w[2], 2); r1 = __shfl_xor_sync(0xffffffffu, b1 ? w[1] : w[3], 2);
+        if (b1) { w[0] = r0; w[1] = r1; } else { w[2] = r0; w[3] = r1; }
+        *reinterpret_cast<float4*>(hs + (int64_t)r * 8 * g.K + 16 * kb + 4 * qt) = make_float4(w[0], w[1], w[2], w[3]);
+      }
+    }
+  };
 #pragma unroll 1
   for (int i = 0; i < my_tiles; ++i) {
 #pragma unroll
     for (int j = 0; j < 128; ++j) acc[j] = 0.f;
     int prev = 0;
-#pragma unroll 1
-    for (int kb = 0; kb < nkb; ++kb) {
+    if constexpr (FUSE) {
+    auto mma_ra = [&](int kb, uint32_t (&fh)[2][4], uint32_t (&fl)[2][4]) {
       mbar_wait(full0 + 8 * s, ph);
+      fence_frags(fh, fl);
       const uint32_t cur = (uint32_t)s * STAGE_BYTES;
       wgmma_fence();
-#pragma unroll
+  #pragma unroll
       for (int kk = 0; kk < BK / 8; ++kk) {
         const uint32_t o = cur + kk * 32;
-        const uint64_t ah = a_desc0 + ((o + A_HI) >> 4), al = a_desc0 + ((o + A_LO) >> 4), bh = b_desc0 + ((o + B_HI) >> 4), bl = b_desc0 + ((o + B_LO) >> 4);
+        const uint64_t bh = b_desc0 + ((o + B_HI) >> 4), bl = b_desc0 + ((o + B_LO) >> 4);
         if (split) {
-          wgmma_tf32(acc, al, bh);
-          wgmma_tf32(acc, ah, bl);
-        }
-        wgmma_tf32(acc, ah, bh);
+          wgmma_tf32_ra(acc, fl[kk], bh);
+          wgmma_tf32_ra(acc, fh[kk], bl);
+        }
+        wgmma_tf32_ra(acc, fh[kk], bh);
       }
       wgmma_commit();
       wgmma_wait<1>();
       if (kb > 0) mbar_arrive(empty0 + 8 * prev);
       prev = s;
       if (++s == N_STAGES) { s = 0; ph ^= 1; }
+    };
+
+      const int t = tile_of(i), grp = t / tiles_m, m0 = (t % tiles_m) * BM;
+      uint32_t fh0[2][4] = {}, fl0[2][4] = {}, fh1[2][4] = {}, fl1[2][4] = {};
+      const uint32_t l1b = l1s0 + (uint32_t)(i & 1) * L1_BUF_BYTES;
+      float* hs = p.l1.store ? p.l1.store + (int64_t)grp * p.l1.store_gs + (int64_t)(m0 + lr) * g.K : nullptr;
+      mbar_wait(l1_full0 + 8 * (i & 1), (i >> 1) & 1);
+      fence_frags(fh0, fl0);
+      fence_frags(fh1, fl1);
+      l1_frag(0, l1b, hs, fh0, fl0);
+#pragma unroll 1
+      for (int kb = 0; kb < nkb; kb += 2) {
+        mma_ra(kb, fh0, fl0);
+        fence_frags(fh1, fl1);
+        l1_frag(kb + 1, l1b, hs, fh1, fl1);
+        mma_ra(kb + 1, fh1, fl1);
+        fence_frags(fh0, fl0);
+        if (kb + 2 < nkb) l1_frag(kb + 2, l1b, hs, fh0, fl0);
+        else mbar_arrive(l1_empty0 + 8 * (i & 1));
+      }
+      if (p.l1.bits) {
+        uint32_t* bo = p.l1.bits + (int64_t)grp * p.l1.bits_gs + (int64_t)(m0 + lr) * (BN / 32) + 2 * qt;
+        *reinterpret_cast<uint2*>(bo) = make_uint2(keep0[0], keep0[1]);
+        *reinterpret_cast<uint2*>(bo + 8 * (BN / 32)) = make_uint2(keep1[0], keep1[1]);
+      }
+    } else {
+#pragma unroll 1
+      for (int kb = 0; kb < nkb; ++kb) {
+        mbar_wait(full0 + 8 * s, ph);
+        const uint32_t cur = (uint32_t)s * STAGE_BYTES;
+        wgmma_fence();
+#pragma unroll
+        for (int kk = 0; kk < BK / 8; ++kk) {
+          const uint32_t o = cur + kk * 32;
+          const uint64_t ah = a_desc0 + ((o + A_HI) >> 4), al = a_desc0 + ((o + A_LO) >> 4), bh = b_desc0 + ((o + B_HI) >> 4), bl = b_desc0 + ((o + B_LO) >> 4);
+          if (split) {
+            wgmma_tf32(acc, al, bh);
+            wgmma_tf32(acc, ah, bl);
+          }
+          wgmma_tf32(acc, ah, bh);
+        }
+        wgmma_commit();
+        wgmma_wait<1>();
+        if (kb > 0) mbar_arrive(empty0 + 8 * prev);
+        prev = s;
+        if (++s == N_STAGES) { s = 0; ph ^= 1; }
+      }
     }
 
     const int t = tile_of(i), grp = t / tiles_m, m0 = (t % tiles_m) * BM;
@@ -445,24 +571,25 @@
   return true;
 }
 
-template <int EPI, bool FUSE = false>
+template <int EPI, int L1K = 0>
 int tc_set_attr() {
-  IL_CUDA(cudaFuncSetAttribute(tc_gemm_kernel<EPI, FUSE>, cudaFuncAttributeMaxDynamicSharedMemorySize, smem_bytes(FUSE)));
+  IL_CUDA(cudaFuncSetAttribute(tc_gemm_kernel<EPI, L1K>, cudaFuncAttributeMaxDynamicSharedMemorySize, smem_bytes(L1K > 0)));
   return 0;
 }
 
 int tc_gemm_init() {
   IL_TRY((tc_set_attr<0>())); IL_TRY((tc_set_attr<1>())); IL_TRY((tc_set_attr<2>())); IL_TRY((tc_set_attr<3>())); IL_TRY((tc_set_attr<4>()));
-  IL_TRY((tc_set_attr<4, true>())); IL_TRY((tc_set_attr<5>())); IL_TRY((tc_set_attr<6>()));
+  IL_TRY((tc_set_attr<4, 11>())); IL_TRY((tc_set_attr<4, 12>())); IL_TRY((tc_set_attr<4, 14>()));
+  IL_TRY((tc_set_attr<4, 15>())); IL_TRY((tc_set_attr<4, 16>())); IL_TRY((tc_set_attr<5>())); IL_TRY((tc_set_attr<6>()));
   return 0;
 }
 
-template <int EPI, bool FUSE = false>
+template <int EPI, int L1K = 0>
 static int tc_launch(il_handle* h, TcParams& p, cudaStream_t stream) {
   const GemmArgs& a = p.g;
   p.tiles_m = a.M / BM;
   const int tiles = a.G * p.tiles_m, wave = h->sm_count >= p.tiles_m ? h->sm_count / p.tiles_m * p.tiles_m : h->sm_count;
-  IL_LAUNCH(h, (tc_gemm_kernel<EPI, FUSE>), tiles < wave ? tiles : wave, THREADS, smem_bytes(FUSE), stream, p);
+  IL_LAUNCH(h, (tc_gemm_kernel<EPI, L1K>), tiles < wave ? tiles : wave, THREADS, smem_bytes(L1K > 0), stream, p);
   return 0;
 }
 
@@ -471,7 +598,8 @@
 }
 
 bool tc_l1_fusable(const il_handle* h, const GemmArgs& a, int x_k) {
-  return h->tc_fuse_l1 && tc_gemm_eligible(a) && x_k >= 1 && x_k <= L1_MAXK && a.K <= L1_ROWS && a.a_kmajor;
+  const bool k_ok = x_k == 11 || x_k == 12 || x_k == 14 || x_k == 15 || x_k == 16;
+  return h->tc_fuse_l1 && tc_gemm_eligible(a) && k_ok && a.K == L1_ROWS && a.a_kmajor;
 }
 
 int launch_tc_gemm_head(il_handle* h, const GemmArgs& a, const float* head_w, const float* head_b, int64_t head_gs, int head_n, float* head_out, int64_t head_out_gs, int store_c,
@@ -483,16 +611,28 @@
   p.head_w = head_w; p.head_b = head_b; p.head_out = head_out; p.head_gs = head_gs; p.head_out_gs = head_out_gs; p.head_n = head_n; p.store_c = store_c;
   p.head_js = BN; p.head_ns = 1;
   double bytes = gemm_algorithmic_bytes(a, store_c != 0) + 4.0 * a.G * (double)a.M * head_n, flops = 2.0 * a.M * a.N * a.K * a.G;
+  if (a.bits_out) bytes += 4.0 * a.G * (double)a.M * (a.N / 32);
   if (l1) {
     IL_CHECK(tc_l1_fusable(h, a, l1->x_k), "tc_gemm_head: first layer not fusable (K0=%d)", l1->x_k);
     IL_CHECK(l1->x && l1->w1 && l1->b1 && (reinterpret_cast<uintptr_t>(l1->b1) & 15) == 0 && l1->gs % 4 == 0, "tc_gemm_head: bad first-layer buffers");
     IL_CHECK(!l1->store || ((reinterpret_cast<uintptr_t>(l1->store) & 15) == 0 && l1->store_gs % 4 == 0), "tc_gemm_head: unaligned hidden store");
+    IL_CHECK(!l1->bits || ((reinterpret_cast<uintptr_t>(l1->bits) & 7) == 0 && l1->bits_gs % 2 == 0), "tc_gemm_head: unaligned hidden sign bits");
     p.l1 = *l1;
     const double gx = (a.G + l1->x_gdiv - 1) / l1->x_gdiv;
-    bytes += -4.0 * a.G * (double)a.M * a.K + 4.0 * (gx * a.M * l1->x_k + (double)a.G * a.K * (l1->x_k + 1)) + (l1->store ? 4.0 * a.G * (double)a.M * a.K : 0.0);
+    bytes += -4.0 * a.G * (double)a.M * a.K + 4.0 * (gx * a.M * l1->x_k + (double)a.G * a.K * (l1->x_k + 1)) + (l1->store ? 4.0 * a.G * (double)a.M * a.K : 0.0) +
+             (l1->bits ? 4.0 * a.G * (double)a.M * (a.K / 32) : 0.0);
     flops += 2.0 * a.G * (double)a.M * a.K * l1->x_k;
   }
-  auto run = [&]() { return l1 ? tc_launch<4, true>(h, p, stream) : tc_launch<4>(h, p, stream); };
+  auto run = [&]() {
+    if (!l1) return tc_launch<4>(h, p, stream);
+    switch (l1->x_k) {
+      case 11: return tc_launch<4, 11>(h, p, stream);
+      case 12: return tc_launch<4, 12>(h, p, stream);
+      case 14: return tc_launch<4, 14>(h, p, stream);
+      case 15: return tc_launch<4, 15>(h, p, stream);
+      default: return tc_launch<4, 16>(h, p, stream);
+    }
+  };
   if (h->profiling) {
     ProfiledLaunch pl;
     IL_TRY(profile_open(h, &pl, flops, bytes, stream));
```

New measurement: 86450 (median of 6 runs). +4.8%, better.
